# joesharratt1229/DT4Image_Restoration

Hardware: NVIDIA B200
Metric: pnp_admm_image_iters_per_sec_256 (higher is better)
Workload: dtype bf16

## Files before the change

dt4image_restoration_b200/_lib.py:

```python
from __future__ import annotations

import ctypes as C
import os
import threading

_HERE = os.path.dirname(os.path.abspath(__file__))
LIB_PATH = os.path.join(_HERE, "csrc", "libpnp_b200.so")

_lib = None
_inited = False
_init_device = None
_lock = threading.Lock()

c_void_p, c_int, c_ll, c_size_t, c_char_p = C.c_void_p, C.c_int, C.c_longlong, C.c_size_t, C.c_char_p

SIGNATURES = {
    "pnp_init": (c_int, []),
    "pnp_last_error": (c_char_p, []),
    "pnp_num_sms": (c_int, []),
    "pnp_abi_version": (c_int, []),
    "pnp_psnr": (c_int, [c_void_p, c_void_p, c_ll, c_void_p, c_int, c_int, c_void_p]),
    "pnp_psnr_allgather": (c_int, [c_void_p, c_void_p, c_ll, c_void_p, c_void_p, c_int, c_int, c_int, c_int, c_int,
                                   c_void_p, C.c_uint, C.c_uint, c_void_p, c_int, c_int, c_void_p]),
    "pnp_ssim_workspace_bytes": (c_size_t, [c_int, c_int, c_int]),
    "pnp_ssim": (c_int, [c_void_p, c_void_p, c_ll, c_void_p, c_void_p, c_int, c_int, c_int, c_void_p]),
    "pnp_fft2c": (c_int, [c_void_p, c_void_p, c_int, c_int, c_int, c_int, c_void_p]),
    "pnp_simulate_measurements": (c_int, [c_void_p, c_ll, c_void_p, c_ll, c_void_p, c_int, c_void_p, c_void_p, c_void_p,
                                          c_void_p, c_int, c_int, c_int, c_void_p]),
    "pnp_cartesian_masks": (c_int, [c_void_p, c_int, c_void_p, c_int, c_void_p, c_int, c_int, c_int, c_void_p]),
    "pnp_radial_masks": (c_int, [c_void_p, c_int, c_void_p, c_void_p, c_void_p, c_int, c_int, c_int, c_void_p]),
    "pnp_variable_density_masks": (c_int, [c_void_p, c_int, c_void_p, c_int, c_int, c_int, c_void_p, c_int, c_int, c_int,
                                           c_void_p]),
    "pnp_residual_real": (c_int, [c_void_p, c_void_p, c_void_p, c_ll, c_void_p]),
    "pnp_prox_workspace_bytes": (c_size_t, [c_int, c_int, c_int]),
    "pnp_prox_dual": (c_int, [c_void_p, c_void_p, c_void_p, c_void_p, c_ll, c_void_p, c_int, c_void_p, c_void_p,
                              c_void_p, c_void_p, c_int, c_int, c_int, c_void_p]),
    "pnp_prox_prepared_supported": (c_int, [c_int, c_int]),
    "pnp_prox_prepared_bytes": (c_int, [c_int, c_int, c_int, c_void_p, c_void_p]),
    "pnp_prox_prepare": (c_int, [c_void_p, c_void_p, c_ll, c_void_p, c_void_p, c_int, c_int, c_int, c_void_p]),
    "pnp_prox_dual_prepared": (c_int, [c_void_p, c_void_p, c_void_p, c_void_p, c_ll, c_void_p, c_int, c_void_p, c_void_p,
                                       c_void_p, c_int, c_int, c_int, c_void_p]),
    "pnp_prox_prepared_kind_async": (c_int, [c_void_p, c_ll, c_int, c_int, c_int, c_void_p, c_void_p]),
    "pnp_prox_dual_prepared_kind": (c_int, [c_void_p, c_void_p, c_void_p, c_void_p, c_ll, c_void_p, c_int, c_void_p,
                                            c_void_p, c_void_p, c_int, c_int, c_int, c_int, c_void_p]),
    "pnp_step_prepared_kind": (c_int, [c_void_p, c_void_p, c_void_p, c_void_p, c_void_p, c_void_p, c_ll, c_void_p, c_int,
                                       c_void_p, c_void_p, c_void_p, c_void_p, c_int, c_void_p]),
    "pnp_step_prepared_active": (c_int, [c_void_p, c_void_p, c_void_p, c_void_p, c_void_p, c_void_p, c_ll, c_void_p, c_int,
                                         c_void_p, c_void_p, c_void_p, c_void_p, c_int, c_void_p, c_void_p]),
    "pnp_step_prepared": (c_int, [c_void_p, c_void_p, c_void_p, c_void_p, c_void_p, c_void_p, c_ll, c_void_p, c_int,
                                  c_void_p, c_void_p, c_void_p, c_void_p, c_void_p]),
    "pnp_unet_num_params": (c_size_t, []),
    "pnp_unet_packed_bytes": (c_size_t, []),
    "pnp_unet_pack_weights": (c_int, [c_void_p, c_void_p, c_void_p]),
    "pnp_unet_workspace_bytes": (c_size_t, [c_int, c_int, c_int]),
    "pnp_unet_plan_create": (c_int, [C.POINTER(c_void_p), c_void_p, c_void_p, c_size_t, c_int, c_int, c_int]),
    "pnp_unet_plan_destroy": (None, [c_void_p]),
    "pnp_unet_forward": (c_int, [c_void_p, c_void_p, c_void_p, c_void_p, c_void_p, c_void_p]),
    "pnp_unet_profile": (c_int, [c_void_p, c_void_p, c_void_p, c_void_p, c_void_p, C.POINTER(C.c_float),
                                 C.POINTER(c_int), C.POINTER(c_int), C.POINTER(c_int)]),
    "pnp_unet_num_launches": (c_int, [c_void_p]),
    "pnp_unet_micro_batch": (c_int, [c_void_p]),
    "pnp_unet_set_workspace_cap": (c_size_t, [c_size_t]),
    "pnp_unet_set_splitk": (c_int, [c_int]),
    "pnp_unet_plan_tensor": (c_int, [c_void_p, c_char_p, C.POINTER(c_size_t), C.POINTER(c_int), C.POINTER(c_int),
                                     C.POINTER(c_int)]),
    "pnp_conv3x3_packed_bytes": (c_size_t, [c_int, c_int]),
    "pnp_conv3x3_bf16": (c_int, [c_void_p, c_int, c_void_p, c_int, c_void_p, c_void_p, c_void_p, c_void_p, c_int,
                                 c_int, c_int, c_int, c_void_p]),
    "pnp_policy_packed_floats": (c_size_t, [c_int, c_int]),
    "pnp_policy_step": (c_int, [c_void_p, c_void_p, c_void_p, c_void_p, c_void_p, c_void_p, c_void_p, c_void_p, c_void_p,
                                C.c_float, C.c_float, C.c_float, c_int, c_int, c_int, c_int, c_void_p]),
    "pnp_policy_encoder_packed_floats": (c_size_t, []),
    "pnp_policy_observe": (c_int, [c_void_p, c_void_p, c_int, c_int, c_void_p, c_void_p, c_void_p, c_void_p, c_void_p,
                                   c_void_p, c_void_p, c_int, c_int, c_int, c_void_p]),
    "pnp_step": (c_int, [c_void_p, c_void_p, c_void_p, c_void_p, c_void_p, c_void_p, c_ll, c_void_p, c_int, c_void_p,
                         c_void_p, c_void_p, c_void_p, c_void_p, c_void_p]),
}


class PnpError(RuntimeError):
    pass


def load() -> C.CDLL:
    global _lib
    with _lock:
        if _lib is None:
            if not os.path.exists(LIB_PATH):
                raise PnpError(
                    f"{LIB_PATH} is missing: build it with `python -m dt4image_restoration_b200.build` "
                    "(there is no CPU fallback)")
            lib = C.CDLL(LIB_PATH)
            for name, (res, args) in SIGNATURES.items():
                fn = getattr(lib, name)
                fn.restype = res
                fn.argtypes = args
            _lib = lib
    return _lib


def lib() -> C.CDLL:
    global _inited
    l = load()
    if not _inited:
        with _lock:
            if not _inited:
                rc = l.pnp_init()
                if rc != 0:
                    raise PnpError(f"pnp_init failed ({rc}): {l.pnp_last_error().decode()}")
                global _init_device
                try:
                    import torch
                    _init_device = torch.cuda.current_device()
                except Exception:
                    _init_device = None
                _inited = True
    return l


def check_device(device) -> None:
    import torch
    lib()
    idx = torch.device(device).index
    cur = torch.cuda.current_device()
    if idx is None:
        idx = cur
    if _init_device is not None and (idx != _init_device or cur != _init_device):
        raise PnpError(f"libpnp_b200 was initialised on cuda:{_init_device}; got a tensor on cuda:{idx} with current device "
                       f"cuda:{cur}.  Use one process per GPU and call torch.cuda.set_device(local_rank) before the first "
                       f"operation (there is no multi-device dispatch inside one process)")


def check(rc: int, what: str = "") -> None:
    if rc != 0:
        msg = load().pnp_last_error().decode()
        raise PnpError(f"{what or 'libpnp_b200'} failed with code {rc}: {msg}")


def stream_ptr() -> int:
    import torch
    return torch.cuda.current_stream().cuda_stream
```

dt4image_restoration_b200/csrc/api.cu:

```cuda
#include <mutex>
#include <string>
#include "../../include/pnp_b200.h"
#include "common.cuh"
#include "pnp_internal.h"

namespace pnp {
static thread_local std::string t_err;
void set_error(const std::string& msg) { t_err = msg; }
static std::once_flag g_once;
static int g_init_rc = -100;

static int fail_cuda(int rc, const char* where) {
  if (rc > 0 && rc < 1000) set_error(std::string(where) + ": " + cudaGetErrorString(cudaError_t(rc)));
  return rc;
}

__global__ void residual_real_kernel(const float2* __restrict__ z, const float2* __restrict__ u, float* __restrict__ v,
                                     long long n) {
  for (long long i = blockIdx.x * (long long)blockDim.x + threadIdx.x; i < n; i += (long long)gridDim.x * blockDim.x)
    v[i] = z[i].x - u[i].x;
}
}

using namespace pnp;

struct pnp_unet_plan {
  UnetPlan* impl;
  UnetPlan* tail;
  int B, H, W, mb;
};

namespace pnp {
static size_t kUnetWorkspaceCap = size_t(8) << 30;
static int unet_micro_batch(int B, int H, int W) {
  if (unet_workspace_bytes(B, H, W) <= kUnetWorkspaceCap) return B;
  const size_t per8 = unet_workspace_bytes(8, H, W);
  long long m = (long long)(kUnetWorkspaceCap / per8) * 8;
  if (m < 1) m = 1;
  while (m > 1 && unet_workspace_bytes(int(m), H, W) > kUnetWorkspaceCap) m -= (m > 8 ? 8 : 1);
  return int(m < B ? m : B);
}
}

extern "C" {

int pnp_abi_version(void) { return 1; }

int pnp_init(void) {
  std::call_once(g_once, [] {
    int dev = 0;
    cudaError_t e = cudaGetDevice(&dev);
    if (e != cudaSuccess) { g_init_rc = int(e); set_error("no CUDA device"); return; }
    cudaDeviceProp prop;
    cudaGetDeviceProperties(&prop, dev);
    if (prop.major != 10) {
      set_error("libpnp_b200 requires an sm_100a (B200) device; found sm_" + std::to_string(prop.major) +
                std::to_string(prop.minor));
      g_init_rc = -10;
      return;
    }
    init_fft_tables();
    int rc = unet_global_init();
    if (rc == 0) rc = int(cudaGetLastError());
    g_init_rc = rc;
  });
  return g_init_rc;
}

const char* pnp_last_error(void) { return t_err.c_str(); }
int pnp_num_sms(void) { return num_sms(); }

#define REQUIRE_INIT()                                          \
  if (g_init_rc != 0) {                                         \
    set_error("pnp_init() has not succeeded");                  \
    return -3;                                                  \
  }

int pnp_psnr(const float* x, const float* gt, long long gt_batch_stride, float* out, int B, int HW, void* stream) {
  REQUIRE_INIT();
  if (!x || !gt || !out) { set_error("pnp_psnr: null pointer"); return -1; }
  return fail_cuda(psnr_launch(x, gt, gt_batch_stride, out, B, HW, cudaStream_t(stream)), "pnp_psnr");
}

int pnp_psnr_allgather(const float* x, const float* gt, long long gt_batch_stride, float* out_local,
                       const unsigned long long* peer_base, int rank, int world, int slot_floats, int parity,
                       int flag_word, unsigned int* local_count, unsigned int count_target, unsigned int flag_target,
                       int* err_flag, int B, int HW, void* stream) {
  REQUIRE_INIT();
  if (!x || !gt || !peer_base || !local_count || !err_flag) { set_error("pnp_psnr_allgather: null pointer"); return -1; }
  if (world < 1 || world > 8 || rank < 0 || rank >= world || B > slot_floats) {
    set_error("pnp_psnr_allgather: need 1 <= world <= 8, 0 <= rank < world, B <= slot_floats");
    return -1;
  }
  return fail_cuda(psnr_allgather_launch(x, gt, gt_batch_stride, out_local, peer_base, rank, world, slot_floats, parity,
                                         flag_word, local_count, count_target, flag_target, err_flag, B, HW,
                                         cudaStream_t(stream)), "pnp_psnr_allgather");
}

size_t pnp_ssim_workspace_bytes(int B, int H, int W) { return ssim_workspace_bytes(B, H, W); }

int pnp_ssim(const float* x, const float* gt, long long gt_batch_stride, float* out, void* workspace, int B, int H, int W,
             void* stream) {
  REQUIRE_INIT();
  if (!x || !gt || !out || !workspace) { set_error("pnp_ssim: null pointer"); return -1; }
  if (B <= 0) { set_error("pnp_ssim: need B > 0"); return -1; }
  if (H < 11 || W < 11) { set_error("pnp_ssim: H and W must be at least 11 (11x11 window, valid filtering)"); return -2; }
  if (reinterpret_cast<uintptr_t>(workspace) & 15) { set_error("pnp_ssim: workspace must be 16-byte aligned"); return -1; }
  return fail_cuda(ssim_launch(x, gt, gt_batch_stride, out, workspace, B, H, W, cudaStream_t(stream)), "pnp_ssim");
}

int pnp_fft2c(const void* src, void* dst, int B, int H, int W, int inverse, void* stream) {
  REQUIRE_INIT();
  if (!src || !dst || B <= 0) { set_error("pnp_fft2c: bad argument"); return -1; }
  if (!fft_any_shape_supported(H, W)) { set_error("pnp_fft2c: H and W must be in [2, 1024]"); return -2; }
  return fail_cuda(fft2c_general(static_cast<const float2*>(src), static_cast<float2*>(dst), B, H, W, inverse,
                                 cudaStream_t(stream)), "pnp_fft2c");
}

static bool ranges_overlap(const void* a, size_t na, const void* b, size_t nb) {
  const uintptr_t pa = reinterpret_cast<uintptr_t>(a), pb = reinterpret_cast<uintptr_t>(b);
  return a && b && pa < pb + nb && pb < pa + na;
}

int pnp_simulate_measurements(const float* gt, long long gt_batch_stride, const uint8_t* mask, long long mask_batch_stride,
                              const float* sigma_n, int sigma_stride, const unsigned long long* seeds, void* y0_out,
                              void* x0_out, void* aty0_out, int B, int H, int W, void* stream) {
  if (!gt || !mask || !sigma_n || !seeds || !y0_out || !x0_out) {
    set_error("pnp_simulate_measurements: null pointer");
    return -1;
  }
  if (B <= 0 || gt_batch_stride < 0 || mask_batch_stride < 0 || sigma_stride < 0) {
    set_error("pnp_simulate_measurements: need B > 0 and non-negative strides");
    return -1;
  }
  if (!fft_any_shape_supported(H, W)) { set_error("pnp_simulate_measurements: H and W must be in [2, 1024]"); return -2; }
  const size_t hw = size_t(H) * W, nout = size_t(B) * hw * sizeof(float2);
  const size_t ngt = (size_t(B - 1) * gt_batch_stride + hw) * sizeof(float);
  const size_t nmask = size_t(B - 1) * mask_batch_stride + hw;
  const void* outs[3] = {y0_out, x0_out, aty0_out};
  for (int k = 0; k < 3; ++k) {
    bool bad = ranges_overlap(outs[k], nout, gt, ngt) || ranges_overlap(outs[k], nout, mask, nmask);
    for (int q = k + 1; q < 3; ++q) bad |= ranges_overlap(outs[k], nout, outs[q], nout);
    if (bad) { set_error("pnp_simulate_measurements: outputs overlap each other, gt or mask"); return -1; }
  }
  REQUIRE_INIT();
  return fail_cuda(simulate_measurements(gt, gt_batch_stride, mask, mask_batch_stride, sigma_n, sigma_stride, seeds,
                                         static_cast<float2*>(y0_out), static_cast<float2*>(x0_out),
                                         static_cast<float2*>(aty0_out), B, H, W, cudaStream_t(stream)),
                   "pnp_simulate_measurements");
}

int pnp_cartesian_masks(const int* accel, int accel_stride, const unsigned long long* seeds, int acs_cols, uint8_t* mask_out,
                        int B, int H, int W, void* stream) {
  if (!accel || !seeds || !mask_out) { set_error("pnp_cartesian_masks: null pointer"); return -1; }
  if (B <= 0 || accel_stride < 0 || acs_cols < 1) {
    set_error("pnp_cartesian_masks: need B > 0, accel_stride >= 0 and acs_cols >= 1");
    return -1;
  }
  if (!fft_any_shape_supported(H, W)) { set_error("pnp_cartesian_masks: H and W must be in [2, 1024]"); return -2; }
  REQUIRE_INIT();
  return fail_cuda(cartesian_masks(accel, accel_stride, seeds, acs_cols, mask_out, B, H, W, cudaStream_t(stream)),
                   "pnp_cartesian_masks");
}

int pnp_radial_masks(const double* frac, int frac_stride, const unsigned long long* seeds, uint8_t* mask_out,
                     int* lines_out, int B, int H, int W, void* stream) {
  if (!frac || !mask_out) { set_error("pnp_radial_masks: null pointer"); return -1; }
  if (B <= 0 || frac_stride < 0) { set_error("pnp_radial_masks: need B > 0 and frac_stride >= 0"); return -1; }
  if (!fft_any_shape_supported(H, W)) { set_error("pnp_radial_masks: H and W must be in [2, 1024]"); return -2; }
  const size_t nmask = size_t(B) * H * W, nlines = size_t(B) * sizeof(int);
  const size_t nfrac = (size_t(B - 1) * frac_stride + 1) * sizeof(double), nseeds = size_t(B) * sizeof(unsigned long long);
  const bool bad = ranges_overlap(lines_out, nlines, mask_out, nmask) || ranges_overlap(mask_out, nmask, frac, nfrac) ||
                   ranges_overlap(mask_out, nmask, seeds, nseeds) || ranges_overlap(lines_out, nlines, frac, nfrac) ||
                   ranges_overlap(lines_out, nlines, seeds, nseeds);
  if (bad) { set_error("pnp_radial_masks: outputs overlap each other, frac or seeds"); return -1; }
  REQUIRE_INIT();
  return fail_cuda(radial_masks(frac, frac_stride, seeds, mask_out, lines_out, B, H, W, cudaStream_t(stream)),
                   "pnp_radial_masks");
}

int pnp_variable_density_masks(const int* accel, int accel_stride, const unsigned long long* seeds, int acs_h, int acs_w,
                               int power, uint8_t* mask_out, int B, int H, int W, void* stream) {
  if (!accel || !seeds || !mask_out) { set_error("pnp_variable_density_masks: null pointer"); return -1; }
  if (B <= 0 || accel_stride < 0) { set_error("pnp_variable_density_masks: need B > 0 and accel_stride >= 0"); return -1; }
  if (!fft_any_shape_supported(H, W)) { set_error("pnp_variable_density_masks: H and W must be in [2, 1024]"); return -2; }
  if (acs_h < 0 || acs_h > H || acs_w < 0 || acs_w > W || power < 0 || power > 16) {
    set_error("pnp_variable_density_masks: need 0 <= acs_h <= H, 0 <= acs_w <= W and 0 <= power <= 16");
    return -1;
  }
  const size_t nmask = size_t(B) * H * W, nseeds = size_t(B) * sizeof(unsigned long long);
  const size_t naccel = (size_t(B - 1) * accel_stride + 1) * sizeof(int);
  if (ranges_overlap(mask_out, nmask, accel, naccel) || ranges_overlap(mask_out, nmask, seeds, nseeds)) {
    set_error("pnp_variable_density_masks: mask_out overlaps accel or seeds");
    return -1;
  }
  REQUIRE_INIT();
  return fail_cuda(variable_density_masks(accel, accel_stride, seeds, acs_h, acs_w, power, mask_out, B, H, W,
                                          cudaStream_t(stream)), "pnp_variable_density_masks");
}

int pnp_residual_real(const void* z, const void* u, float* v, long long n, void* stream) {
  REQUIRE_INIT();
  long long g = (n + 255) / 256;
  if (g > 148 * 16) g = 148 * 16;
  if (g < 1) g = 1;
  residual_real_kernel<<<int(g), 256, 0, cudaStream_t(stream)>>>(static_cast<const float2*>(z),
                                                                 static_cast<const float2*>(u), v, n);
  return fail_cuda(int(cudaGetLastError()), "pnp_residual_real");
}

size_t pnp_prox_workspace_bytes(int B, int H, int W) { return size_t(B) * H * W * (sizeof(float2) + 1); }

int pnp_prox_prepared_supported(int H, int W) { return fft_shape_supported(H, W); }

int pnp_prox_prepared_bytes(int B, int H, int W, size_t* y0p_bytes, size_t* maskp_bytes) {
  if (!y0p_bytes || !maskp_bytes || B <= 0) { set_error("pnp_prox_prepared_bytes: bad argument"); return -1; }
  if (!pnp_prox_prepared_supported(H, W)) { set_error("pnp_prox_prepared_bytes: H and W must be powers of two in 32..512"); return -2; }
  prox_prepared_bytes(B, H, W, y0p_bytes, maskp_bytes);
  return 0;
}

int pnp_prox_prepare(const void* y0, const uint8_t* mask, long long mask_batch_stride, void* y0T, uint8_t* maskT, int B,
                     int H, int W, void* stream) {
  REQUIRE_INIT();
  if (!y0 || !mask || !y0T || !maskT) { set_error("pnp_prox_prepare: null pointer"); return -1; }
  if (!pnp_prox_prepared_supported(H, W)) { set_error("pnp_prox_prepare: H and W must be powers of two in 32..512"); return -2; }
  return fail_cuda(prox_prepare(static_cast<const float2*>(y0), mask, mask_batch_stride, static_cast<float2*>(y0T), maskT,
                                B, H, W, cudaStream_t(stream)), "pnp_prox_prepare");
}

int pnp_prox_prepared_kind_async(const uint8_t* maskT, long long mask_batch_stride, int B, int H, int W, int* kind_host,
                                 void* stream) {
  REQUIRE_INIT();
  if (!maskT || !kind_host) { set_error("pnp_prox_prepared_kind_async: null pointer"); return -1; }
  if (!pnp_prox_prepared_supported(H, W)) { set_error("pnp_prox_prepared_kind_async: unsupported shape"); return -2; }
  return fail_cuda(int(cudaMemcpyAsync(kind_host, prox_prepared_flag(maskT, mask_batch_stride, B, H, W), sizeof(int),
                                       cudaMemcpyDeviceToHost, cudaStream_t(stream))), "pnp_prox_prepared_kind_async");
}

int pnp_prox_dual_prepared(const float* x, const void* u_in, const void* y0T, const uint8_t* maskT,
                           long long mask_batch_stride, const float* mu, int mu_stride, void* z_out, void* u_out,
                           float* v_next, int B, int H, int W, void* stream) {
  return pnp_prox_dual_prepared_kind(x, u_in, y0T, maskT, mask_batch_stride, mu, mu_stride, z_out, u_out, v_next, B, H, W,
                                     -1, stream);
}

int pnp_prox_dual_prepared_kind(const float* x, const void* u_in, const void* y0T, const uint8_t* maskT,
                                long long mask_batch_stride, const float* mu, int mu_stride, void* z_out, void* u_out,
                                float* v_next, int B, int H, int W, int kind, void* stream) {
  REQUIRE_INIT();
  if (kind < -1 || kind > 1) { set_error("pnp_prox_dual_prepared_kind: kind must be -1, 0 or 1"); return -1; }
  if (!x || !u_in || !y0T || !maskT || !mu || !z_out || !u_out) { set_error("pnp_prox_dual_prepared: null pointer"); return -1; }
  if (!pnp_prox_prepared_supported(H, W)) { set_error("pnp_prox_dual_prepared: H and W must be powers of two in 32..512"); return -2; }
  return fail_cuda(prox_dual_prepared(x, static_cast<const float2*>(u_in), static_cast<const float2*>(y0T), maskT,
                                      mask_batch_stride, mu, mu_stride, static_cast<float2*>(z_out),
                                      static_cast<float2*>(u_out), v_next, B, H, W, kind, cudaStream_t(stream)),
                   "pnp_prox_dual_prepared");
}

int pnp_prox_dual(const float* x, const void* u_in, const void* y0, const uint8_t* mask, long long mask_batch_stride,
                  const float* mu, int mu_stride, void* z_out, void* u_out, float* v_next, void* workspace, int B,
                  int H, int W, void* stream) {
  REQUIRE_INIT();
  if (!x || !u_in || !y0 || !mask || !mu || !z_out || !u_out || !workspace) {
    set_error("pnp_prox_dual: null pointer");
    return -1;
  }
  if (!fft_any_shape_supported(H, W)) {
    set_error("pnp_prox_dual: H and W must be in [2, 1024]");
    return -2;
  }
  return fail_cuda(prox_dual_general(x, static_cast<const float2*>(u_in), static_cast<const float2*>(y0), mask,
                                     mask_batch_stride, mu, mu_stride, static_cast<float2*>(z_out),
                                     static_cast<float2*>(u_out), v_next, static_cast<float2*>(workspace), B, H, W,
                                     cudaStream_t(stream)), "pnp_prox_dual");
}

size_t pnp_unet_num_params(void) { return unet_num_params(); }
size_t pnp_unet_packed_bytes(void) { return unet_packed_bytes(); }
size_t pnp_unet_workspace_bytes(int B, int H, int W) {
  if (B <= 0 || H <= 0 || W <= 0) return 0;
  return unet_workspace_bytes(unet_micro_batch(B, H, W), H, W);
}

int pnp_unet_pack_weights(const float* flat_params, void* packed, void* stream) {
  REQUIRE_INIT();
  return fail_cuda(unet_pack(flat_params, static_cast<uint8_t*>(packed), cudaStream_t(stream)), "pnp_unet_pack_weights");
}

int pnp_unet_plan_create(pnp_unet_plan** plan, const void* packed, void* workspace, size_t workspace_bytes, int B,
                         int H, int W) {
  REQUIRE_INIT();
  if (B <= 0) { set_error("pnp_unet_plan_create: B must be positive"); return -1; }
  const int mb = unet_micro_batch(B, H, W);
  UnetPlan *impl = nullptr, *tail = nullptr;
  int rc = unet_plan_create(&impl, static_cast<const uint8_t*>(packed), static_cast<uint8_t*>(workspace),
                            workspace_bytes, mb, H, W);
  if (rc) return rc;
  if (B % mb) {
    rc = unet_plan_create(&tail, static_cast<const uint8_t*>(packed), static_cast<uint8_t*>(workspace), workspace_bytes,
                          B % mb, H, W);
    if (rc) { unet_plan_destroy(impl); return rc; }
  }
  *plan = new pnp_unet_plan{impl, tail, B, H, W, mb};
  return 0;
}

void pnp_unet_plan_destroy(pnp_unet_plan* plan) {
  if (!plan) return;
  unet_plan_destroy(plan->impl);
  if (plan->tail) unet_plan_destroy(plan->tail);
  delete plan;
}

int pnp_unet_forward(pnp_unet_plan* plan, const float* v, const float* sigma, float* x_out, float* preclamp,
                     void* stream) {
  REQUIRE_INIT();
  if (!plan || !v || !sigma || !x_out) { set_error("pnp_unet_forward: null pointer"); return -1; }
  const size_t hw = size_t(plan->H) * plan->W;
  for (int i0 = 0; i0 < plan->B; i0 += plan->mb) {
    UnetPlan* p = (plan->B - i0 >= plan->mb) ? plan->impl : plan->tail;
    int rc = unet_forward(p, v + i0 * hw, sigma + i0, x_out + i0 * hw, preclamp ? preclamp + i0 * hw : nullptr,
                          cudaStream_t(stream));
    if (rc) return fail_cuda(rc, "pnp_unet_forward");
  }
  return 0;
}

int pnp_unet_profile(pnp_unet_plan* plan, const float* v, const float* sigma, float* x_out, void* stream, float* ms,
                     int* kinds, int* ids, int* n_inout) {
  REQUIRE_INIT();
  if (!plan || !v || !sigma || !x_out || !ms || !kinds || !ids || !n_inout) {
    set_error("pnp_unet_profile: null pointer");
    return -1;
  }
  const size_t hw = size_t(plan->H) * plan->W;
  const int cap = *n_inout;
  int used = 0;
  for (int i0 = 0; i0 < plan->B; i0 += plan->mb) {
    UnetPlan* p = (plan->B - i0 >= plan->mb) ? plan->impl : plan->tail;
    int n = cap - used;
    int rc = unet_profile(p, v + i0 * hw, sigma + i0, x_out + i0 * hw, cudaStream_t(stream), ms + used, kinds + used,
                          ids + used, &n);
    if (rc) return fail_cuda(rc, "pnp_unet_profile");
    used += n;
  }
  *n_inout = used;
  return 0;
}

int pnp_unet_num_launches(const pnp_unet_plan* plan) {
  if (!plan) return -1;
  return (plan->B / plan->mb) * unet_num_launches(plan->impl) + (plan->tail ? unet_num_launches(plan->tail) : 0);
}

int pnp_unet_micro_batch(const pnp_unet_plan* plan) { return plan ? plan->mb : -1; }

size_t pnp_unet_set_workspace_cap(size_t bytes) {
  const size_t old = kUnetWorkspaceCap;
  if (bytes) kUnetWorkspaceCap = bytes;
  return old;
}

int pnp_unet_set_splitk(int mode) { return unet_set_splitk(mode); }

int pnp_unet_plan_tensor(const pnp_unet_plan* plan, const char* name, size_t* byte_offset, int* C, int* H, int* W) {
  if (!plan || !name) return -1;
  if (plan->mb != plan->B) return -1;
  return unet_plan_tensor(plan->impl, name, byte_offset, C, H, W);
}

size_t pnp_policy_packed_floats(int n_time, int n_task) { return policy_packed_floats(n_time, n_task); }

int pnp_policy_step(const float* packed, const float* rtg, const float* emb, float* act, const long long* timesteps,
                    const long long* task, const long long* pos, float* act_out, float* rtg_out, float scale0, float scale1,
                    float scale2, int B, int K, int n_time, int n_task, void* stream) {
  REQUIRE_INIT();
  if (!packed || !rtg || !emb || !act || !timesteps || !task || !pos || !act_out || !rtg_out) {
    set_error("pnp_policy_step: null pointer");
    return -1;
  }
  if (K < 1 || K > 6 || B < 1) { set_error("pnp_policy_step: need 1 <= K <= 6 context entries and B >= 1"); return -1; }
  return fail_cuda(policy_step_launch(packed, rtg, emb, act, timesteps, task, pos, act_out, rtg_out, scale0, scale1, scale2,
                                      B, K, n_time, n_task, cudaStream_t(stream)), "pnp_policy_step");
}

size_t pnp_policy_encoder_packed_floats(void) { return policy_encoder_packed_floats(); }

int pnp_policy_observe(const float* enc_packed, const float* x, int H, int W, const float* next_rtg, float* rtg, float* emb,
                       float* act, long long* timesteps, const long long* pos, const long long* t_dev, int B, int K,
                       int n_time, void* stream) {
  if (!enc_packed || !x || !next_rtg || !rtg || !emb || !act || !timesteps || !pos || !t_dev) {
    set_error("pnp_policy_observe: null pointer");
    return -1;
  }
  if (K < 1 || K > 6 || B < 1 || H != W || H < 128 || H % 128 != 0 || n_time < 1) {
    set_error("pnp_policy_observe: need square images whose edge is a multiple of 128, 1 <= K <= 6 and B >= 1");
    return -1;
  }
  return fail_cuda(policy_observe_launch(enc_packed, x, H, W, next_rtg, rtg, emb, act, timesteps, pos, t_dev, B, K, n_time,
                                         cudaStream_t(stream)), "pnp_policy_observe");
}

size_t pnp_conv3x3_packed_bytes(int Cin, int Cout) { return (conv_packed_bytes(Cin, Cout) + 1023) / 1024 * 1024; }

int pnp_conv3x3_bf16(const void* in0, int C0, const void* in1, int C1, const float* weights, const float* bias,
                     void* out, void* scratch, int B, int H, int W, int Cout, void* stream) {
  REQUIRE_INIT();
  return fail_cuda(conv3x3_single(static_cast<const __nv_bfloat16*>(in0), C0, static_cast<const __nv_bfloat16*>(in1),
                                  C1, weights, bias, static_cast<__nv_bfloat16*>(out), static_cast<uint8_t*>(scratch),
                                  B, H, W, Cout, cudaStream_t(stream)), "pnp_conv3x3_bf16");
}

int pnp_step_prepared(pnp_unet_plan* plan, const float* v, const float* sigma, const void* u_in, const void* y0T,
                      const uint8_t* maskT, long long mask_batch_stride, const float* mu, int mu_stride, float* x_out,
                      void* z_out, void* u_out, float* v_next, void* stream) {
  return pnp_step_prepared_kind(plan, v, sigma, u_in, y0T, maskT, mask_batch_stride, mu, mu_stride, x_out, z_out, u_out,
                                v_next, -1, stream);
}

int pnp_step_prepared_kind(pnp_unet_plan* plan, const float* v, const float* sigma, const void* u_in, const void* y0T,
                           const uint8_t* maskT, long long mask_batch_stride, const float* mu, int mu_stride, float* x_out,
                           void* z_out, void* u_out, float* v_next, int kind, void* stream) {
  int rc = pnp_unet_forward(plan, v, sigma, x_out, nullptr, stream);
  if (rc) return rc;
  return pnp_prox_dual_prepared_kind(x_out, u_in, y0T, maskT, mask_batch_stride, mu, mu_stride, z_out, u_out, v_next,
                                     plan->B, plan->H, plan->W, kind, stream);
}

int pnp_step_prepared_active(pnp_unet_plan* plan, const float* v, const float* sigma, const void* u_in, const void* y0T,
                             const uint8_t* maskT, long long mask_batch_stride, const float* mu, int mu_stride,
                             float* x_out, void* z_out, void* u_out, float* v_next, int kind, const uint8_t* active,
                             void* stream) {
  REQUIRE_INIT();
  if (!plan || !v || !sigma || !u_in || !y0T || !maskT || !mu || !x_out || !z_out || !u_out) {
    set_error("pnp_step_prepared_active: null pointer");
    return -1;
  }
  if (kind < -1 || kind > 1) { set_error("pnp_step_prepared_active: kind must be -1, 0 or 1"); return -1; }
  const size_t hw = size_t(plan->H) * plan->W;
  for (int i0 = 0; i0 < plan->B; i0 += plan->mb) {
    UnetPlan* p = (plan->B - i0 >= plan->mb) ? plan->impl : plan->tail;
    int rc = unet_forward(p, v + i0 * hw, sigma + i0, x_out + i0 * hw, nullptr, cudaStream_t(stream),
                          active ? active + i0 : nullptr);
    if (rc) return fail_cuda(rc, "pnp_step_prepared_active");
  }
  return fail_cuda(prox_dual_prepared(x_out, static_cast<const float2*>(u_in), static_cast<const float2*>(y0T), maskT,
                                      mask_batch_stride, mu, mu_stride, static_cast<float2*>(z_out),
                                      static_cast<float2*>(u_out), v_next, plan->B, plan->H, plan->W, kind,
                                      cudaStream_t(stream), active), "pnp_step_prepared_active");
}

int pnp_step(pnp_unet_plan* plan, const float* v, const float* sigma, const void* u_in, const void* y0,
             const uint8_t* mask, long long mask_batch_stride, const float* mu, int mu_stride, float* x_out,
             void* z_out, void* u_out, float* v_next, void* prox_workspace, void* stream) {
  int rc = pnp_unet_forward(plan, v, sigma, x_out, nullptr, stream);
  if (rc) return rc;
  return pnp_prox_dual(x_out, u_in, y0, mask, mask_batch_stride, mu, mu_stride, z_out, u_out, v_next, prox_workspace,
                       plan->B, plan->H, plan->W, stream);
}

}
```

dt4image_restoration_b200/csrc/pnp_internal.h:

```cpp
#pragma once
#include <cuda_runtime.h>
#include <cuda_bf16.h>
#include <stddef.h>
#include <stdint.h>
#include <string>

namespace pnp {

void set_error(const std::string& msg);

int psnr_launch(const float* x, const float* gt, long long gt_bstride, float* out, int B, int HW, cudaStream_t st);
int psnr_allgather_launch(const float* x, const float* gt, long long gt_bstride, float* out_local,
                          const unsigned long long* peer_base, int rank, int world, int slot, int parity, int flag_word,
                          unsigned int* local_count, unsigned int count_target, unsigned int flag_target, int* err,
                          int B, int HW, cudaStream_t st);

size_t ssim_workspace_bytes(int B, int H, int W);
int ssim_launch(const float* x, const float* gt, long long gt_bstride, float* out, void* workspace, int B, int H, int W,
                cudaStream_t st);

void init_fft_tables();
int fft_shape_supported(int H, int W);
int fft_any_shape_supported(int H, int W);
int prox_dual_general(const float* x, const float2* u_in, const float2* y0, const uint8_t* mask,
                      long long mask_bstride, const float* mu, int mu_stride, float2* z_out, float2* u_out,
                      float* v_out, float2* work, int B, int H, int W, cudaStream_t st);
void prox_prepared_bytes(int B, int H, int W, size_t* y0p_bytes, size_t* maskp_bytes);
int prox_prepare(const float2* y0, const uint8_t* mask, long long mask_bstride, float2* y0T, uint8_t* maskT, int B, int H,
                 int W, cudaStream_t st);
int prox_dual_prepared(const float* x, const float2* u_in, const float2* y0T, const uint8_t* maskT,
                       long long mask_bstride, const float* mu, int mu_stride, float2* z_out, float2* u_out,
                       float* v_out, int B, int H, int W, int kind, cudaStream_t st, const uint8_t* active = nullptr);
const int* prox_prepared_flag(const uint8_t* maskp, long long mask_bstride, int B, int H, int W);
int fft2c_general(const float2* src, float2* dst, int B, int H, int W, int inverse, cudaStream_t st);
int simulate_measurements(const float* gt, long long gt_bstride, const uint8_t* mask, long long mask_bstride,
                          const float* sigma, int sigma_stride, const unsigned long long* seeds, float2* y0, float2* x0,
                          float2* aty0, int B, int H, int W, cudaStream_t st);
int cartesian_masks(const int* accel, int accel_stride, const unsigned long long* seeds, int acs_cols, uint8_t* mask,
                    int B, int H, int W, cudaStream_t st);
int radial_masks(const double* frac, int frac_stride, const unsigned long long* seeds, uint8_t* mask, int* lines_out,
                 int B, int H, int W, cudaStream_t st);
int variable_density_masks(const int* accel, int accel_stride, const unsigned long long* seeds, int acs_h, int acs_w,
                           int power, uint8_t* mask, int B, int H, int W, cudaStream_t st);

size_t policy_packed_floats(int n_time, int n_task);
int policy_step_launch(const float* w, const float* rtg, const float* emb, float* act, const long long* ts,
                       const long long* task, const long long* pos, float* act_out, float* rtg_out, float s0, float s1,
                       float s2, int B, int K, int n_time, int n_task, cudaStream_t st);
size_t policy_encoder_packed_floats();
int policy_observe_launch(const float* w, const float* x, int H, int W, const float* nxt_rtg, float* w_rtg, float* w_emb,
                          float* w_act, long long* w_ts, const long long* pos, const long long* t_dev, int B, int K,
                          int n_time, cudaStream_t st);

struct UnetPlan;
int unet_global_init();
int num_sms();
size_t unet_num_params();
size_t unet_packed_bytes();
size_t unet_workspace_bytes(int B, int H, int W);
int unet_pack(const float* flat_fp32, uint8_t* packed, cudaStream_t st);
int unet_plan_create(UnetPlan** out, const uint8_t* packed, uint8_t* workspace, size_t workspace_bytes, int B, int H,
                     int W);
void unet_plan_destroy(UnetPlan* p);
int unet_plan_tensor(const UnetPlan* p, const char* name, size_t* off, int* C, int* H, int* W);
int unet_forward(UnetPlan* p, const float* v, const float* sigma, float* x_out, float* preclamp, cudaStream_t st,
                 const uint8_t* active = nullptr);
int unet_profile(UnetPlan* p, const float* v, const float* sigma, float* x_out, cudaStream_t st, float* ms, int* kinds,
                 int* ids, int* n_inout);
int unet_num_launches(const UnetPlan* p);
int unet_set_splitk(int mode);
size_t conv_packed_bytes(int Cin, int Cout);
int conv3x3_single(const __nv_bfloat16* in0, int C0, const __nv_bfloat16* in1, int C1, const float* w_fp32,
                   const float* bias, __nv_bfloat16* out, uint8_t* wpk_scratch, int B, int H, int W, int Cout,
                   cudaStream_t st);

}
```

dt4image_restoration_b200/csrc/unet.cu:

```cuda
#include <algorithm>
#include <mutex>
#include <vector>
#include <string>
#include <cstring>
#include "common.cuh"
#include "unet_conv.cuh"
#include "unet_conv_kws.cuh"
#include "unet_conv_pair.cuh"
#include "unet_conv_splitk.cuh"
#include "pnp_internal.h"

namespace pnp {

struct FirstConvW {
  float w[9][32];
  float b[32];
  float ws[9][32];
};


__global__ void __launch_bounds__(256) conv_first_kernel(const float* __restrict__ v, const float* __restrict__ sigma,
                                                         const __grid_constant__ FirstConvW cw,
                                                         __nv_bfloat16* __restrict__ out, int B, int H, int W,
                                                         float slope, int rev, int ppt) {
  grid_dep_launch();
  grid_dep_wait();
  const int x = blockIdx.x * blockDim.x + threadIdx.x;
  const int pairs = (H + 1) / 2;
  const int pair0 = ppt * (rev ? int(gridDim.y) - 1 - int(blockIdx.y) : int(blockIdx.y));
  const int pair1 = pair0 + ppt < pairs ? pair0 + ppt : pairs;
  const int b = rev ? B - 1 - int(blockIdx.z) : int(blockIdx.z);
  if (x >= W) return;
  const float sg = __ldg(sigma + b);
  const float* vb = v + size_t(b) * H * W + x;
  const bool xl = x > 0, xr = x + 1 < W;
  const int cx = xl ? (xr ? 1 : 2) : 0;
  auto load_row = [&](int yy, float (&r)[3]) {
    const bool ok = (yy >= 0) && (yy < H);
    const float* row = vb + ptrdiff_t(yy) * W;
    r[0] = (ok && xl) ? __ldg(row - 1) : 0.f;
    r[1] = ok ? __ldg(row) : 0.f;
    r[2] = (ok && xr) ? __ldg(row + 1) : 0.f;
  };
  float in[4][3], nx[2][3];
#pragma unroll
  for (int r = 0; r < 4; ++r) load_row(2 * pair0 - 1 + r, in[r]);
#pragma unroll 1
  for (int pair = pair0; pair < pair1; ++pair) {
    const int y0 = 2 * pair;
    load_row(y0 + 3, nx[0]);
    load_row(y0 + 4, nx[1]);
    const int cs0 = (y0 == 0 ? 0 : (y0 == H - 1 ? 6 : 3)) + cx;
    const int cs1 = (y0 + 1 == H - 1 ? 6 : 3) + cx;
    float acc0[32], acc1[32];
    if (cs0 == 4 && cs1 == 4) {
#pragma unroll
      for (int co = 0; co < 32; ++co) acc0[co] = acc1[co] = fmaf(sg, cw.ws[4][co], cw.b[co]);
    } else {
#pragma unroll
      for (int co = 0; co < 32; ++co) {
        acc0[co] = fmaf(sg, cw.ws[cs0][co], cw.b[co]);
        acc1[co] = fmaf(sg, cw.ws[cs1][co], cw.b[co]);
      }
    }
#pragma unroll
    for (int t = 0; t < 9; ++t) {
#pragma unroll
      for (int co = 0; co < 32; ++co) {
        const float wv = cw.w[t][co];
        acc0[co] = fmaf(wv, in[t / 3][t % 3], acc0[co]);
        acc1[co] = fmaf(wv, in[t / 3 + 1][t % 3], acc1[co]);
      }
    }
#pragma unroll
    for (int p = 0; p < 2; ++p) {
      if (p == 1 && y0 + 1 >= H) break;
      const float* acc = p ? acc1 : acc0;
      uint32_t o[16];
#pragma unroll
      for (int co = 0; co < 32; co += 2) {
        const float a0 = fmaxf(acc[co], acc[co] * slope);
        const float a1 = fmaxf(acc[co + 1], acc[co + 1] * slope);
        o[co / 2] = pack_bf16x2(a0, a1);
      }
      uint4* dst = reinterpret_cast<uint4*>(out + ((size_t(b) * H + y0 + p) * W + x) * 32);
      dst[0] = make_uint4(o[0], o[1], o[2], o[3]);
      dst[1] = make_uint4(o[4], o[5], o[6], o[7]);
      dst[2] = make_uint4(o[8], o[9], o[10], o[11]);
      dst[3] = make_uint4(o[12], o[13], o[14], o[15]);
    }
#pragma unroll
    for (int c = 0; c < 3; ++c) {
      in[0][c] = in[2][c]; in[1][c] = in[3][c]; in[2][c] = nx[0][c]; in[3][c] = nx[1][c];
    }
  }
}


constexpr int kUpsRows = 4;
__global__ void __launch_bounds__(256) upsample2x_kernel(const uint4* __restrict__ in, uint4* __restrict__ out, int B,
                                                         int h, int w, int Ho, int Wo, int C8, int py, int px,
                                                         float sy, float sx) {
  grid_dep_launch();
  grid_dep_wait();
  const int e = blockIdx.x * blockDim.x + threadIdx.x;
  if (e >= Wo * C8) return;
  const int c = e % C8, xo = e / C8;
  const int b = blockIdx.z;
  const int ux = xo - px;
  const bool xin = ux >= 0 && ux < 2 * w;
  const float fx = sx * float(ux);
  const int x0 = xin ? int(fx) : 0;
  const int x1 = x0 + (x0 < w - 1 ? 1 : 0);
  const float lx = fx - float(x0), hx = 1.f - lx;
  const size_t base = size_t(b) * h * w;
  uint4 q[kUpsRows][4];
  float ly[kUpsRows];
  bool ok[kUpsRows];
#pragma unroll
  for (int r = 0; r < kUpsRows; ++r) {
    const int yo = blockIdx.y * kUpsRows + r;
    const int uy = yo - py;
    ok[r] = xin && yo < Ho && uy >= 0 && uy < 2 * h;
    const float fy = sy * float(uy);
    const int y0 = ok[r] ? int(fy) : 0;
    const int y1 = y0 + (y0 < h - 1 ? 1 : 0);
    ly[r] = fy - float(y0);
    q[r][0] = __ldg(in + (base + size_t(y0) * w + x0) * C8 + c);
    q[r][1] = __ldg(in + (base + size_t(y0) * w + x1) * C8 + c);
    q[r][2] = __ldg(in + (base + size_t(y1) * w + x0) * C8 + c);
    q[r][3] = __ldg(in + (base + size_t(y1) * w + x1) * C8 + c);
  }
#pragma unroll
  for (int r = 0; r < kUpsRows; ++r) {
    const int yo = blockIdx.y * kUpsRows + r;
    if (yo >= Ho) break;
    uint4 res = make_uint4(0, 0, 0, 0);
    if (ok[r]) {
      const float hy = 1.f - ly[r];
      const __nv_bfloat162* a = reinterpret_cast<const __nv_bfloat162*>(&q[r][0]);
      const __nv_bfloat162* bq = reinterpret_cast<const __nv_bfloat162*>(&q[r][1]);
      const __nv_bfloat162* cq = reinterpret_cast<const __nv_bfloat162*>(&q[r][2]);
      const __nv_bfloat162* d = reinterpret_cast<const __nv_bfloat162*>(&q[r][3]);
      uint32_t* o = reinterpret_cast<uint32_t*>(&res);
#pragma unroll
      for (int k = 0; k < 4; ++k) {
        const float2 f00 = __bfloat1622float2(a[k]), f01 = __bfloat1622float2(bq[k]);
        const float2 f10 = __bfloat1622float2(cq[k]), f11 = __bfloat1622float2(d[k]);
        const float vx = hy * (hx * f00.x + lx * f01.x) + ly[r] * (hx * f10.x + lx * f11.x);
        const float vy = hy * (hx * f00.y + lx * f01.y) + ly[r] * (hx * f10.y + lx * f11.y);
        o[k] = pack_bf16x2(vx, vy);
      }
    }
    out[(size_t(b) * Ho + yo) * Wo * C8 + e] = res;
  }
}

__device__ __forceinline__ float small_int_to_float(int k) { return __int_as_float(0x4B000000 + (k + 1)) - 8388609.0f; }


__global__ void __launch_bounds__(256) upsample2x_fast_kernel(const uint4* __restrict__ in, uint4* __restrict__ out,
                                                              int h, int w, int C8, float sy, float sx, int nimg,
                                                              int rev, int c8_shift, int walk) {
  grid_dep_launch();
  grid_dep_wait();
  const int e = blockIdx.x * blockDim.x + threadIdx.x;
  if (e >= (w + 1) * C8) return;
  const int c = e & (C8 - 1), n = (e >> c8_shift) - 1;
  const int by = rev ? int(gridDim.y) - 1 - int(blockIdx.y) : int(blockIdx.y);
  const int m0 = by * walk - 1;
  const int m1 = (m0 + walk < h) ? m0 + walk : h;
  const int b = rev ? nimg - 1 - int(blockIdx.z) : int(blockIdx.z);
  const int xa = n < 0 ? 0 : n, xb = n + 1 < w ? n + 1 : w - 1;
  const uint4* src = in + size_t(b) * h * w * C8 + c;
  const int Ho = 2 * h, Wo = 2 * w;
  float lx[2];
#pragma unroll
  for (int j = 0; j < 2; ++j) lx[j] = sx * small_int_to_float(2 * n + 1 + j) - small_int_to_float(n);
  auto xlerp = [&](const uint4& qa, const uint4& qb, float2 (&t)[2][4]) {
    const uint32_t* a = reinterpret_cast<const uint32_t*>(&qa);
    const uint32_t* bb = reinterpret_cast<const uint32_t*>(&qb);
#pragma unroll
    for (int k = 0; k < 4; ++k) {
      const float2 fa = make_float2(__uint_as_float(a[k] << 16), __uint_as_float(a[k] & 0xffff0000u));
      const float2 fb = make_float2(__uint_as_float(bb[k] << 16), __uint_as_float(bb[k] & 0xffff0000u));
#pragma unroll
      for (int j = 0; j < 2; ++j) {
        const float2 l2 = make_float2(lx[j], lx[j]), h2 = make_float2(1.f - lx[j], 1.f - lx[j]);
        t[j][k] = __ffma2_rn(fb, l2, __fmul2_rn(fa, h2));
      }
    }
  };
  auto row_ptr = [&](int y) { return src + size_t(y < 0 ? 0 : (y < h ? y : h - 1)) * w * C8; };
  float2 top[2][4], bot[2][4];
  {
    const uint4* r = row_ptr(m0);
    xlerp(__ldg(r + size_t(xa) * C8), __ldg(r + size_t(xb) * C8), top);
  }
  const uint4* rn = row_ptr(m0 + 1);
  uint4 qa = __ldg(rn + size_t(xa) * C8), qb = __ldg(rn + size_t(xb) * C8);
#pragma unroll 1
  for (int m = m0; m < m1; ++m) {
    xlerp(qa, qb, bot);
    if (m + 1 < m1) {
      rn = row_ptr(m + 2);
      qa = __ldg(rn + size_t(xa) * C8); qb = __ldg(rn + size_t(xb) * C8);
    }
#pragma unroll
    for (int i = 0; i < 2; ++i) {
      const int yo = 2 * m + 1 + i;
      if (yo < 0 || yo >= Ho) continue;
      const float ly = sy * small_int_to_float(yo) - small_int_to_float(m);
      const float2 ll = make_float2(ly, ly), hh = make_float2(1.f - ly, 1.f - ly);
#pragma unroll
      for (int j = 0; j < 2; ++j) {
        const int xo = 2 * n + 1 + j;
        if (xo < 0 || xo >= Wo) continue;
        uint4 res;
#pragma unroll
        for (int k = 0; k < 4; ++k) {
          const float2 v = __ffma2_rn(bot[j][k], ll, __fmul2_rn(top[j][k], hh));
          reinterpret_cast<uint32_t*>(&res)[k] = pack_bf16x2(v.x, v.y);
        }
        out[((size_t(b) * Ho + yo) * Wo + xo) * C8 + c] = res;
      }
    }
#pragma unroll
    for (int j = 0; j < 2; ++j)
#pragma unroll
      for (int k = 0; k < 4; ++k) top[j][k] = bot[j][k];
  }
}

__global__ void pack_weights_kernel(const float* __restrict__ w, uint8_t* __restrict__ out, int Cin, int Cout, int KC,
                                    int BN) {
  const int n_tiles = Cout / BN;
  const int ROWB = KC * 2;
  const int swz_mask = (ROWB == 128) ? 7 : 3;
  const size_t total = size_t(Cout) * Cin * 9;
  for (size_t i = size_t(blockIdx.x) * blockDim.x + threadIdx.x; i < total; i += size_t(gridDim.x) * blockDim.x) {
    const int tap = int(i % 9);
    const int ci = int((i / 9) % Cin);
    const int co = int(i / (size_t(9) * Cin));
    const int chunk = ci / KC, kk = ci % KC;
    const int nt = co / BN, n = co % BN;
    const uint32_t off = uint32_t(n * ROWB + (kk / 8) * 16);
    const uint32_t phys = off ^ (((off >> 7) & swz_mask) << 4);
    const size_t blob = (size_t(chunk) * 9 + tap) * n_tiles + nt;
    __nv_bfloat16* dst = reinterpret_cast<__nv_bfloat16*>(out + blob * size_t(BN) * ROWB + phys) + (kk % 8);
    *dst = __float2bfloat16_rn(w[i]);
  }
}

__global__ void pack_weights_kws_kernel(const float* __restrict__ w, uint8_t* __restrict__ out, int Cin) {
  const size_t total = size_t(32) * Cin * 9;
  for (size_t i = size_t(blockIdx.x) * blockDim.x + threadIdx.x; i < total; i += size_t(gridDim.x) * blockDim.x) {
    const int tap = int(i % 9), kh = tap / 3, kw = tap % 3;
    const int ci = int((i / 9) % Cin);
    const int co = int(i / (size_t(9) * Cin));
    const int chunk = ci / 32, kk = ci % 32;
    const int n = kw * 32 + co;
    const uint32_t off = uint32_t(n * 64 + (kk / 8) * 16);
    const uint32_t phys = off ^ (((off >> 7) & 3) << 4);
    const size_t blob = size_t(chunk) * 3 + kh;
    __nv_bfloat16* dst = reinterpret_cast<__nv_bfloat16*>(out + blob * size_t(KwsCfg::B_BYTES) + phys) + (kk % 8);
    *dst = __float2bfloat16_rn(w[i]);
  }
}

typedef CUresult (*EncodeTiledFn)(CUtensorMap*, CUtensorMapDataType, cuuint32_t, void*, const cuuint64_t*,
                                  const cuuint64_t*, const cuuint32_t*, const cuuint32_t*, CUtensorMapInterleave,
                                  CUtensorMapSwizzle, CUtensorMapL2promotion, CUtensorMapFloatOOBfill);
static EncodeTiledFn g_encode = nullptr;
static int g_num_sms = 148;
static const int kSkGain = 3;
static int g_splitk_mode = -1;
int unet_set_splitk(int mode) {
  const int old = g_splitk_mode;
  if (mode >= -1 && mode <= 1) g_splitk_mode = mode;
  return old;
}

static const int kConvSmemMax = 227 * 1024;
static const int kConvSmemBudget = 222 * 1024;

template <int KC, int BN, int EPI>
static int set_conv_attr() {
  return int(cudaFuncSetAttribute(conv3x3_umma_kernel<KC, BN, EPI>, cudaFuncAttributeMaxDynamicSharedMemorySize,
                                  kConvSmemMax));
}

int unet_global_init() {
  void* fn = nullptr;
  cudaDriverEntryPointQueryResult qres;
  cudaError_t e = cudaGetDriverEntryPoint("cuTensorMapEncodeTiled", &fn, cudaEnableDefault, &qres);
  if (e != cudaSuccess || fn == nullptr) {
    set_error("cuTensorMapEncodeTiled driver entry point not available");
    return e != cudaSuccess ? int(e) : 999;
  }
  g_encode = reinterpret_cast<EncodeTiledFn>(fn);
  int dev = 0;
  cudaGetDevice(&dev);
  cudaDeviceGetAttribute(&g_num_sms, cudaDevAttrMultiProcessorCount, dev);
  int rc = 0;
  rc |= set_conv_attr<32, 32, EPI_BF16>();
  rc |= set_conv_attr<32, 32, EPI_FINAL>();
  rc |= set_conv_attr<32, 64, EPI_BF16>();
  rc |= set_conv_attr<64, 64, EPI_BF16>();
  rc |= set_conv_attr<64, 128, EPI_BF16>();
  rc |= int(cudaFuncSetAttribute(conv3x3_pair_kernel<32, 64>, cudaFuncAttributeMaxDynamicSharedMemorySize, kConvSmemMax));
  rc |= int(cudaFuncSetAttribute(conv3x3_pair_kernel<64, 64>, cudaFuncAttributeMaxDynamicSharedMemorySize, kConvSmemMax));
  rc |= int(cudaFuncSetAttribute(conv3x3_pair_kernel<64, 128>, cudaFuncAttributeMaxDynamicSharedMemorySize, kConvSmemMax));
  rc |= int(cudaFuncSetAttribute(conv3x3_kws_kernel, cudaFuncAttributeMaxDynamicSharedMemorySize, kConvSmemMax));
  rc |= int(cudaFuncSetAttribute(conv3x3_splitk_kernel, cudaFuncAttributeMaxDynamicSharedMemorySize, kSkSmem));
  if (rc) set_error("cudaFuncSetAttribute(MaxDynamicSharedMemorySize) failed");
  return rc;
}

int num_sms() { return g_num_sms; }

static int make_act_map(CUtensorMap* m, const void* base, int B, int H, int W, int C, int KC, int box_w = kHalo,
                        int box_h = kHalo) {
  if (!g_encode) { set_error("pnp_init() has not been called"); return -3; }
  cuuint64_t dims[4] = {cuuint64_t(C), cuuint64_t(W), cuuint64_t(H), cuuint64_t(B)};
  cuuint64_t strides[3] = {cuuint64_t(C) * 2, cuuint64_t(W) * C * 2, cuuint64_t(H) * W * C * 2};
  cuuint32_t box[4] = {cuuint32_t(KC), cuuint32_t(box_w), cuuint32_t(box_h), 1};
  cuuint32_t estr[4] = {1, 1, 1, 1};
  CUresult r = g_encode(m, CU_TENSOR_MAP_DATA_TYPE_BFLOAT16, 4, const_cast<void*>(base), dims, strides, box, estr,
                        CU_TENSOR_MAP_INTERLEAVE_NONE, KC == 64 ? CU_TENSOR_MAP_SWIZZLE_128B : CU_TENSOR_MAP_SWIZZLE_64B,
                        CU_TENSOR_MAP_L2_PROMOTION_L2_128B, CU_TENSOR_MAP_FLOAT_OOB_FILL_NONE);
  if (r != CUDA_SUCCESS) {
    set_error("cuTensorMapEncodeTiled failed (code " + std::to_string(int(r)) + ")");
    return 1000 + int(r);
  }
  return 0;
}

struct ConvLaunch {
  ConvParams p;
  CUtensorMap tm0, tm1;
  CUtensorMap tmw;
  int KC, BN, EPI;
  int kws;
  int pair;
  int splitk;
  int grid;
  int smem;
};

static const int kConvBarBytes = (4 * 16 + 2 * 4 + 2) * 8 + 16 + kEpiSmemFloats * 4;
static const int kConvRingBytes = kConvSmemBudget - 1024 - kConvBarBytes - 1024;
static int halo_stage_bytes(int KC) { return (kHalo * kHalo * KC * 2 + 1023) / 1024 * 1024; }

static bool weights_fit(int KC, int n_tiles, long long wbytes) {
  return n_tiles == 1 && wbytes + 3 * halo_stage_bytes(KC) <= kConvRingBytes;
}

static void size_rings(ConvLaunch& L) {
  if (L.kws) {
    const int bar = KwsCfg::BAR_BYTES;
    const int avail = kConvSmemBudget - 1024 - bar - 1024;
    const int wtotal = (L.p.nchunks0 + L.p.nchunks1) * 3 * KwsCfg::B_BYTES;
    int sa = (avail - wtotal) / KwsCfg::A_STAGE;
    L.p.wres = 1; L.p.sb = 1;
    L.p.sa = sa > 8 ? 8 : sa;
    L.smem = 1024 + L.p.sa * KwsCfg::A_STAGE + ((wtotal + 1023) & ~1023) + bar;
    return;
  }
  const int ROWB = L.KC * 2;
  const int a_stage = halo_stage_bytes(L.KC);
  const int b_bytes = L.BN * ROWB / (L.pair ? 2 : 1);
  const int b_stage = (b_bytes + 1023) / 1024 * 1024;
  const int bar = kConvBarBytes;
  const int avail = kConvRingBytes;
  const int nchunks = L.p.nchunks0 + L.p.nchunks1;
  const int wtotal = nchunks * 9 * b_bytes;
  ConvParams& p = L.p;
  if (weights_fit(L.KC, p.n_tiles, wtotal)) {
    p.wres = 1;
    p.sb = 1;
    int sa = (avail - wtotal) / a_stage;
    p.sa = sa > 8 ? 8 : sa;
    L.smem = 1024 + p.sa * a_stage + ((wtotal + 1023) & ~1023) + bar;
  } else {
    p.wres = 0;
    p.sa = 2;
    int sb = (avail - p.sa * a_stage) / b_stage;
    if (sb > 12) sb = 12;
    if (sb < 2) { p.sa = 2; sb = (avail - p.sa * a_stage) / b_stage; }
    p.sb = sb;
    L.smem = 1024 + p.sa * a_stage + p.sb * b_stage + bar;
  }
}

static int pick_bn(int Cout) { return Cout >= 128 ? 128 : Cout; }

static bool use_kws(int C0, int C1, int Cout) {
  return Cout == 32 && C0 > 0 && C0 % 32 == 0 && C1 % 32 == 0 && (C0 + C1) >= 64 && (C0 + C1) <= 96;
}

size_t conv_packed_bytes(int Cin, int Cout) { return size_t(Cin) * Cout * 9 * 2; }

static int build_conv(ConvLaunch& L, const __nv_bfloat16* in0, int C0, const __nv_bfloat16* in1, int C1,
                      const uint8_t* wpk, const float* bias, __nv_bfloat16* out, int B, int H, int W, int Cout,
                      int epi) {
  const bool kws = use_kws(C0, C1, Cout);
  const int KC = (!kws && C0 % 64 == 0 && C1 % 64 == 0) ? 64 : 32;
  if (C0 % KC || C1 % KC || C0 <= 0) { set_error("conv: channel counts must be multiples of 32"); return -4; }
  const int BN = pick_bn(Cout);
  if (Cout % BN) { set_error("conv: Cout must be 32, 64 or a multiple of 128"); return -4; }
  if (epi == EPI_FINAL && !(KC == 32 && BN == 32)) { set_error("conv: FINAL epilogue needs Cin=Cout=32"); return -4; }
  L = ConvLaunch{};
  L.KC = KC; L.BN = BN; L.EPI = epi; L.kws = kws ? 1 : 0;
  {
    static const int pair_env = [] { const char* e = getenv("PNP_CONV_PAIR"); return e ? atoi(e) : -1; }();
    const bool eligible = !kws && epi == EPI_BF16 && (BN == 64 || BN == 128);
    const bool want = pair_env < 0 ? !weights_fit(KC, Cout / BN, (long long)(C0 + C1) * 9 * BN * 2) : pair_env == 1;
    L.pair = (eligible && want) ? 1 : 0;
  }
  ConvParams& p = L.p;
  {
    const long long pix_tiles = (long long)B * ((W + kTile - 1) / kTile) * ((H + kTile - 1) / kTile);
    const bool eligible = !kws && epi == EPI_BF16 && KC == 64 && Cout % kSkBN == 0;
    const long long units = pix_tiles * (Cout / kSkBN);
    if (eligible && g_splitk_mode != 0 && (units <= g_num_sms || g_splitk_mode == 1) && units < (1ll << 24)) {
      const int nch = (C0 + C1) / kSkKC;
      int S = 8;
      while (S > 1 && (nch % S != 0 || units * S > g_num_sms)) S >>= 1;
      const long long reg_ctas = std::min<long long>(pix_tiles * (Cout / BN), g_num_sms);
      if (g_splitk_mode == 1 || units * S >= kSkGain * reg_ctas) {
        L.splitk = 1; L.pair = 0;
        p.sk_split = S; p.sk_cpc = nch / S; p.sk_stages = p.sk_cpc < kSkStages ? p.sk_cpc : kSkStages;
      }
    }
  }
  p.B = B; p.H = H; p.W = W;
  p.tiles_x = kws ? (W + kKwsTileW - 1) / kKwsTileW : (W + kTile - 1) / kTile;
  p.tiles_y = kws ? (H + kKwsTileH - 1) / kKwsTileH : (H + kTile - 1) / kTile;
  p.n_tiles = Cout / BN;
  p.nchunks0 = C0 / KC; p.nchunks1 = C1 / KC;
  p.Cout = Cout; p.wpk = wpk; p.bias = bias; p.out = out; p.slope = 0.2f;
  p.mg_n = conv_magic(uint32_t(p.n_tiles)); p.mg_x = conv_magic(uint32_t(p.tiles_x)); p.mg_y = conv_magic(uint32_t(p.tiles_y));
  {
    const long long tiles_all = (long long)B * p.tiles_x * p.tiles_y * p.n_tiles;
    const int dmax = std::max(p.n_tiles, std::max(p.tiles_x, p.tiles_y));
    if (tiles_all * dmax >= (1ll << 32) || Cout > 512) { set_error("conv: problem too large for the tile index arithmetic"); return -4; }
  }
  size_rings(L);
  const int bw = kws ? kKwsHaloW : kHalo, bh = kws ? kKwsHaloH : kHalo;
  int rc = make_act_map(&L.tm0, in0, B, H, W, C0, KC, bw, bh);
  if (rc) return rc;
  rc = C1 > 0 ? make_act_map(&L.tm1, in1, B, H, W, C1, KC, bw, bh) : make_act_map(&L.tm1, in0, B, H, W, C0, KC, bw, bh);
  if (rc) return rc;
  if (L.pair) {
    const cuuint64_t rows = cuuint64_t(p.nchunks0 + p.nchunks1) * 9 * Cout;
    cuuint64_t dims[2] = {cuuint64_t(KC), rows};
    cuuint64_t strides[1] = {cuuint64_t(KC) * 2};
    cuuint32_t box[2] = {cuuint32_t(KC), cuuint32_t(BN / 2)};
    cuuint32_t estr[2] = {1, 1};
    CUresult r = g_encode(&L.tmw, CU_TENSOR_MAP_DATA_TYPE_BFLOAT16, 2, const_cast<uint8_t*>(wpk), dims, strides, box, estr,
                          CU_TENSOR_MAP_INTERLEAVE_NONE, CU_TENSOR_MAP_SWIZZLE_NONE, CU_TENSOR_MAP_L2_PROMOTION_L2_128B,
                          CU_TENSOR_MAP_FLOAT_OOB_FILL_NONE);
    if (r != CUDA_SUCCESS) { set_error("cuTensorMapEncodeTiled (weights) failed (code " + std::to_string(int(r)) + ")"); return 1000 + int(r); }
  }
  long long tiles = (long long)B * p.tiles_x * p.tiles_y * p.n_tiles;
  if (L.pair) {
    const long long pix = (long long)B * p.tiles_x * p.tiles_y;
    tiles = (pix + 1) / 2 * p.n_tiles;
    p.total_tiles = int(tiles);
    const long long pairs = g_num_sms / 2;
    L.grid = 2 * int(tiles < pairs ? tiles : pairs);
  } else {
  p.total_tiles = int(tiles);
  L.grid = int(tiles < g_num_sms ? tiles : g_num_sms);
  }
  if (L.splitk) {
    L.grid = int((long long)B * p.tiles_x * p.tiles_y * (Cout / kSkBN) * p.sk_split);
    L.smem = sk_smem_bytes(p.sk_stages);
  }
  return 0;
}

template <typename... KArgs, typename... Args>
static cudaError_t launch_k(void (*kernel)(KArgs...), dim3 grid, dim3 block, size_t smem, cudaStream_t st, Args&&... args) {
  cudaLaunchConfig_t cfg{};
  cfg.gridDim = grid; cfg.blockDim = block; cfg.dynamicSmemBytes = smem; cfg.stream = st;
  cudaLaunchAttribute attr[1];
  attr[0].id = cudaLaunchAttributeProgrammaticStreamSerialization;
  attr[0].val.programmaticStreamSerializationAllowed = 1;
  cfg.attrs = attr;
  cfg.numAttrs = 1;
  return cudaLaunchKernelEx(&cfg, kernel, KArgs(args)...);
}

template <int KC, int BN, int EPI>
static void launch_conv_t(const ConvLaunch& L, cudaStream_t st) {
  launch_k(conv3x3_umma_kernel<KC, BN, EPI>, dim3(L.grid), dim3(kConvThreads), size_t(L.smem), st, L.p, L.tm0, L.tm1);
}

static int launch_conv(const ConvLaunch& L, cudaStream_t st) {
  if (L.splitk) {
    cudaLaunchConfig_t cfg{};
    cfg.gridDim = dim3(L.grid); cfg.blockDim = dim3(kConvThreads); cfg.dynamicSmemBytes = size_t(L.smem); cfg.stream = st;
    cudaLaunchAttribute attr[2];
    attr[0].id = cudaLaunchAttributeClusterDimension;
    attr[0].val.clusterDim.x = unsigned(L.p.sk_split); attr[0].val.clusterDim.y = 1; attr[0].val.clusterDim.z = 1;
    attr[1].id = cudaLaunchAttributeProgrammaticStreamSerialization;
    attr[1].val.programmaticStreamSerializationAllowed = 1;
    cfg.attrs = attr; cfg.numAttrs = 2;
    return int(cudaLaunchKernelEx(&cfg, conv3x3_splitk_kernel, L.p, L.tm0, L.tm1));
  }
  if (L.pair) {
    if (L.KC == 32 && L.BN == 64)
      launch_k(conv3x3_pair_kernel<32, 64>, dim3(L.grid), dim3(kConvThreads), size_t(L.smem), st, L.p, L.tm0, L.tm1, L.tmw);
    else if (L.KC == 64 && L.BN == 64)
      launch_k(conv3x3_pair_kernel<64, 64>, dim3(L.grid), dim3(kConvThreads), size_t(L.smem), st, L.p, L.tm0, L.tm1, L.tmw);
    else if (L.KC == 64 && L.BN == 128)
      launch_k(conv3x3_pair_kernel<64, 128>, dim3(L.grid), dim3(kConvThreads), size_t(L.smem), st, L.p, L.tm0, L.tm1, L.tmw);
    else { set_error("conv: unsupported (KC,BN) combination for the pair kernel"); return -4; }
    return int(cudaGetLastError());
  }
  if (L.kws) {
    launch_k(conv3x3_kws_kernel, dim3(L.grid), dim3(kConvThreads), size_t(L.smem), st, L.p, L.tm0, L.tm1);
    return int(cudaGetLastError());
  }
  if (L.EPI == EPI_FINAL) launch_conv_t<32, 32, EPI_FINAL>(L, st);
  else if (L.KC == 32 && L.BN == 32) launch_conv_t<32, 32, EPI_BF16>(L, st);
  else if (L.KC == 32 && L.BN == 64) launch_conv_t<32, 64, EPI_BF16>(L, st);
  else if (L.KC == 64 && L.BN == 64) launch_conv_t<64, 64, EPI_BF16>(L, st);
  else if (L.KC == 64 && L.BN == 128) launch_conv_t<64, 128, EPI_BF16>(L, st);
  else { set_error("conv: unsupported (KC,BN) combination"); return -4; }
  return int(cudaGetLastError());
}

static int ew_grid(size_t total) {
  size_t g = (total + 255) / 256;
  const size_t cap = size_t(g_num_sms) * 16;
  return int(g < cap ? (g ? g : 1) : cap);
}

int pack_conv_weights(const float* w_fp32, uint8_t* out, int Cin, int Cout, int KC, cudaStream_t st, bool kws) {
  if (kws) {
    pack_weights_kws_kernel<<<ew_grid(size_t(Cin) * Cout * 9), 256, 0, st>>>(w_fp32, out, Cin);
    return int(cudaGetLastError());
  }
  const int BN = pick_bn(Cout);
  pack_weights_kernel<<<ew_grid(size_t(Cin) * Cout * 9), 256, 0, st>>>(w_fp32, out, Cin, Cout, KC, BN);
  return int(cudaGetLastError());
}

int conv3x3_single(const __nv_bfloat16* in0, int C0, const __nv_bfloat16* in1, int C1, const float* w_fp32,
                   const float* bias, __nv_bfloat16* out, uint8_t* wpk_scratch, int B, int H, int W, int Cout,
                   cudaStream_t st) {
  ConvLaunch L;
  int rc = build_conv(L, in0, C0, in1, C1, wpk_scratch, bias, out, B, H, W, Cout, EPI_BF16);
  if (rc) return rc;
  rc = pack_conv_weights(w_fp32, wpk_scratch, C0 + C1, Cout, L.KC, st, L.kws != 0);
  if (rc) return rc;
  return launch_conv(L, st);
}

static const int kCh[5] = {32, 64, 128, 256, 512};

struct TensorSlot { size_t off; int C, H, W; };

enum { K_FIRST = 0, K_UMMA = 1, K_UPS = 3 };

struct Op {
  int kind;
  int id;
  int level;
  int conv;
  int rev;
};

struct UnetPlan {
  int B, H, W;
  int Hl[5], Wl[5];
  uint8_t* ws;
  size_t ws_bytes;
  const uint8_t* wts;
  TensorSlot tA[5], tB[5], skip[5], pooled[5], ups[4];
  std::vector<ConvLaunch> convs;
  std::vector<Op> ops;
  FirstConvW first;
};

struct LayerDesc { int cin, cout; size_t w_off, b_off; size_t pk_off; };
static const int kBlockCin[9] = {2, 32, 64, 128, 256, 768, 384, 192, 96};
static const int kBlockCout[9] = {32, 64, 128, 256, 512, 256, 128, 64, 32};

static void layer_table(LayerDesc (&L)[27], size_t& outc_w, size_t& outc_b, size_t& n_params, size_t& pk_bytes) {
  size_t off = 0, pk = 0;
  for (int blk = 0; blk < 9; ++blk)
    for (int i = 0; i < 3; ++i) {
      LayerDesc& d = L[blk * 3 + i];
      d.cin = (i == 0) ? kBlockCin[blk] : kBlockCout[blk];
      d.cout = kBlockCout[blk];
      d.w_off = off; off += size_t(d.cout) * d.cin * 9;
      d.b_off = off; off += d.cout;
      d.pk_off = pk;
      if (blk * 3 + i > 0) pk += (conv_packed_bytes(d.cin, d.cout) + 1023) / 1024 * 1024;
    }
  outc_w = off; off += 32;
  outc_b = off; off += 1;
  n_params = off;
  pk_bytes = pk;
}

size_t unet_num_params() {
  LayerDesc L[27]; size_t a, b, n, pk;
  layer_table(L, a, b, n, pk);
  return n;
}
size_t unet_packed_bytes() {
  LayerDesc L[27]; size_t a, b, n, pk;
  layer_table(L, a, b, n, pk);
  return pk + (n * sizeof(float) + 1023) / 1024 * 1024;
}

int unet_pack(const float* flat_fp32, uint8_t* packed, cudaStream_t st) {
  LayerDesc L[27]; size_t ow, ob, n, pk;
  layer_table(L, ow, ob, n, pk);
  for (int i = 1; i < 27; ++i) {
    const int cin = L[i].cin, cout = L[i].cout;
    int c0 = cin, c1 = 0;
    if (i >= 15 && i % 3 == 0) { c0 = kBlockCout[i / 3]; c1 = cin - c0; }
    const bool kws = use_kws(c0, c1, cout);
    const int KC = (!kws && c0 % 64 == 0 && c1 % 64 == 0) ? 64 : 32;
    int rc = pack_conv_weights(flat_fp32 + L[i].w_off, packed + L[i].pk_off, cin, cout, KC, st, kws);
    if (rc) return rc;
  }
  return int(cudaMemcpyAsync(packed + pk, flat_fp32, n * sizeof(float), cudaMemcpyDeviceToDevice, st));
}

static size_t plan_layout(UnetPlan* P) {
  size_t off = 0;
  auto take = [&](TensorSlot& s, int C, int H, int W) {
    s.off = off; s.C = C; s.H = H; s.W = W;
    off += (size_t(P->B) * H * W * C * 2 + 1023) / 1024 * 1024;
  };
  for (int l = 0; l < 5; ++l) {
    take(P->tA[l], kCh[l], P->Hl[l], P->Wl[l]);
    take(P->tB[l], kCh[l], P->Hl[l], P->Wl[l]);
    take(P->skip[l], kCh[l], P->Hl[l], P->Wl[l]);
    if (l > 0) take(P->pooled[l], kCh[l - 1], P->Hl[l], P->Wl[l]);
    if (l < 4) take(P->ups[l], kCh[l + 1], P->Hl[l], P->Wl[l]);
  }
  return off;
}

size_t unet_workspace_bytes(int B, int H, int W) {
  UnetPlan P{};
  P.B = B; P.H = H; P.W = W;
  for (int l = 0; l < 5; ++l) { P.Hl[l] = H >> l; P.Wl[l] = W >> l; }
  return plan_layout(&P);
}

int unet_plan_create(UnetPlan** out, const uint8_t* packed, uint8_t* workspace, size_t workspace_bytes, int B, int H,
                     int W) {
  if (B <= 0 || H < 16 || W < 16) { set_error("unet plan: need B>0 and H,W >= 16"); return -1; }
  UnetPlan* P = new UnetPlan();
  P->B = B; P->H = H; P->W = W;
  for (int l = 0; l < 5; ++l) { P->Hl[l] = H >> l; P->Wl[l] = W >> l; }
  const size_t need = plan_layout(P);
  if (workspace_bytes < need) { delete P; set_error("unet plan: workspace too small"); return -5; }
  if ((reinterpret_cast<uintptr_t>(workspace) & 1023) || (reinterpret_cast<uintptr_t>(packed) & 1023)) {
    delete P; set_error("unet plan: workspace / packed weights must be 1024-byte aligned"); return -6;
  }
  P->ws = workspace; P->ws_bytes = workspace_bytes; P->wts = packed;
  LayerDesc L[27]; size_t ow, ob, n, pk;
  layer_table(L, ow, ob, n, pk);
  const float* flat = reinterpret_cast<const float*>(packed + pk);
  auto T = [&](const TensorSlot& s) { return reinterpret_cast<__nv_bfloat16*>(P->ws + s.off); };
  int rc = 0;
  auto conv = [&](int li, const TensorSlot& in0, const TensorSlot* in1, const TensorSlot& o, int lvl,
                  const TensorSlot* pooled = nullptr) {
    if (rc) return;
    ConvLaunch cl;
    const int epi = (li == 26) ? EPI_FINAL : EPI_BF16;
    rc = build_conv(cl, T(in0), in0.C, in1 ? T(*in1) : nullptr, in1 ? in1->C : 0, packed + L[li].pk_off,
                    flat + L[li].b_off, T(o), B, P->Hl[lvl], P->Wl[lvl], L[li].cout, epi);
    if (rc) return;
    if (epi == EPI_FINAL) { cl.p.wout = flat + ow; cl.p.bout = flat + ob; }
    if (pooled) cl.p.pool_out = T(*pooled);
    P->convs.push_back(cl);
    P->ops.push_back(Op{K_UMMA, li, lvl, int(P->convs.size()) - 1});
  };
  {
    float hw[32 * 18 + 32];
    cudaError_t e = cudaMemcpy(hw, flat + L[0].w_off, sizeof(hw), cudaMemcpyDeviceToHost);
    if (e != cudaSuccess) { delete P; set_error("unet plan: cannot read first-layer weights"); return int(e); }
    for (int co = 0; co < 32; ++co) {
      for (int k = 0; k < 9; ++k) P->first.w[k][co] = hw[co * 18 + k];
      P->first.b[co] = hw[32 * 18 + co];
      for (int cy = 0; cy < 3; ++cy)
        for (int cx = 0; cx < 3; ++cx) {
          float t = 0.f;
          for (int k = 0; k < 9; ++k) {
            const int dy = k / 3 - 1, dx = k % 3 - 1;
            const bool in_y = !((cy == 0 && dy < 0) || (cy == 2 && dy > 0));
            const bool in_x = !((cx == 0 && dx < 0) || (cx == 2 && dx > 0));
            if (in_y && in_x) t += hw[co * 18 + 9 + k];
          }
          P->first.ws[cy * 3 + cx][co] = t;
        }
    }
  }
  P->ops.push_back(Op{K_FIRST, 0, 0, -1});
  conv(1, P->tA[0], nullptr, P->tB[0], 0);
  conv(2, P->tB[0], nullptr, P->skip[0], 0, &P->pooled[1]);
  for (int l = 1; l <= 4; ++l) {
    conv(l * 3 + 0, P->pooled[l], nullptr, P->tA[l], l);
    conv(l * 3 + 1, P->tA[l], nullptr, P->tB[l], l);
    conv(l * 3 + 2, P->tB[l], nullptr, P->skip[l], l, l < 4 ? &P->pooled[l + 1] : nullptr);
  }
  for (int l = 3; l >= 0; --l) {
    const int blk = 5 + (3 - l);
    P->ops.push_back(Op{K_UPS, 200 + l, l, -1});
    conv(blk * 3 + 0, P->skip[l], &P->ups[l], P->tA[l], l);
    conv(blk * 3 + 1, P->tA[l], nullptr, P->tB[l], l);
    conv(blk * 3 + 2, P->tB[l], nullptr, P->tA[l], l);
  }
  if (rc) { delete P; return rc; }
  {
    int k = 0;
    for (Op& op : P->ops) {
      op.rev = k & 1;
      if (op.kind == K_UMMA) P->convs[op.conv].p.rev = op.rev;
      ++k;
    }
  }
  *out = P;
  return 0;
}

void unet_plan_destroy(UnetPlan* P) { delete P; }

int unet_plan_tensor(const UnetPlan* P, const char* name, size_t* off, int* C, int* H, int* W) {
  const TensorSlot* s = nullptr;
  const std::string n(name);
  if (n == "inc.conv-0") s = &P->tA[0];
  else if (n == "inc.conv-1") s = &P->tB[0];
  else if (n == "inc.conv-2") s = &P->skip[0];
  else {
    for (int l = 1; l <= 4 && !s; ++l) {
      const std::string d = "down" + std::to_string(l);
      if (n == d + ".pooled") s = &P->pooled[l];
      else if (n == d + ".conv-0") s = &P->tA[l];
      else if (n == d + ".conv-1") s = &P->tB[l];
      else if (n == d + ".conv-2") s = &P->skip[l];
    }
    for (int k = 1; k <= 4 && !s; ++k) {
      const int l = 4 - k;
      const std::string u = "up" + std::to_string(k);
      if (n == u + ".upsampled") s = &P->ups[l];
    }
  }
  if (!s) return -1;
  *off = s->off; *C = s->C; *H = s->H; *W = s->W;
  return 0;
}

struct ProfileCtx {
  std::vector<cudaEvent_t> ev;
  cudaStream_t st;
  void begin() {
    cudaEvent_t a, b;
    cudaEventCreate(&a); cudaEventCreate(&b);
    ev.push_back(a); ev.push_back(b);
    cudaEventRecord(a, st);
  }
  void end() { cudaEventRecord(ev.back(), st); }
};

static int unet_forward_impl(UnetPlan* P, const float* v, const float* sigma, float* x_out, float* preclamp,
                             cudaStream_t st, ProfileCtx* prof, const uint8_t* active = nullptr) {
  LayerDesc L[27]; size_t ow, ob, n, pk;
  layer_table(L, ow, ob, n, pk);
  auto T = [&](const TensorSlot& s) { return reinterpret_cast<__nv_bfloat16*>(P->ws + s.off); };
  int rc = 0;
  for (const Op& op : P->ops) {
    if (prof) prof->begin();
    switch (op.kind) {
      case K_FIRST: {
        const int bd = P->W >= 256 ? 256 : ((P->W + 31) / 32) * 32;
        const int gx = (P->W + bd - 1) / bd, pairs = (P->H + 1) / 2;
        int ppt = 4;
        while (ppt > 1 && size_t(gx) * ((pairs + ppt - 1) / ppt) * P->B < 4 * 148) ppt >>= 1;
        launch_k(conv_first_kernel, dim3(gx, (pairs + ppt - 1) / ppt, P->B), dim3(bd), 0, st, v, sigma, P->first,
                 T(P->tA[0]), P->B, P->H, P->W, 0.2f, op.rev, ppt);
        break;
      }
      case K_UMMA: {
        ConvLaunch& cl = P->convs[op.conv];
        if (cl.EPI == EPI_FINAL) { cl.p.noisy = v; cl.p.x_out = x_out; cl.p.preclamp = preclamp; cl.p.active = active; }
        rc = launch_conv(cl, st);
        break;
      }
      case K_UPS: {
        const int l = op.level;
        const TensorSlot& lo = (l == 3) ? P->skip[4] : P->tA[l + 1];
        const int h = P->Hl[l + 1], w = P->Wl[l + 1], Ho = P->Hl[l], Wo = P->Wl[l];
        const int C8 = kCh[l + 1] / 8;
        const int dy = Ho - 2 * h, dx = Wo - 2 * w;
        const float sy = (2 * h > 1) ? float(h - 1) / float(2 * h - 1) : 0.f;
        const float sx = (2 * w > 1) ? float(w - 1) / float(2 * w - 1) : 0.f;
        if (dy == 0 && dx == 0 && h > 1 && w > 1)
        {
          const int gx = ((w + 1) * C8 + 255) / 256;
          int walk = 8;
          while (walk > 1 && size_t(gx) * ((h + walk) / walk) * P->B < 4 * size_t(g_num_sms)) walk >>= 1;
          launch_k(upsample2x_fast_kernel, dim3(gx, (h + walk) / walk, P->B), dim3(256), 0, st,
                   reinterpret_cast<const uint4*>(T(lo)), reinterpret_cast<uint4*>(T(P->ups[l])), h, w,
                   C8, sy, sx, P->B, op.rev, (C8 == 64 ? 6 : (C8 == 32 ? 5 : (C8 == 16 ? 4 : 3))), walk);
        }
        else
          launch_k(upsample2x_kernel, dim3((Wo * C8 + 255) / 256, (Ho + kUpsRows - 1) / kUpsRows, P->B), dim3(256), 0,
                   st, reinterpret_cast<const uint4*>(T(lo)), reinterpret_cast<uint4*>(T(P->ups[l])),
                   P->B, h, w, Ho, Wo, C8, dy / 2, dx / 2, sy, sx);
        break;
      }
    }
    if (prof) prof->end();
    if (rc) return rc;
  }
  return int(cudaGetLastError());
}

int unet_forward(UnetPlan* P, const float* v, const float* sigma, float* x_out, float* preclamp, cudaStream_t st,
                 const uint8_t* active) {
  return unet_forward_impl(P, v, sigma, x_out, preclamp, st, nullptr, active);
}

int unet_num_launches(const UnetPlan* P) { return int(P->ops.size()); }

int unet_profile(UnetPlan* P, const float* v, const float* sigma, float* x_out, cudaStream_t st, float* ms,
                 int* kinds, int* ids, int* n_inout) {
  ProfileCtx prof;
  prof.st = st;
  int rc = unet_forward_impl(P, v, sigma, x_out, nullptr, st, &prof);
  cudaError_t e = cudaStreamSynchronize(st);
  const int n = int(prof.ev.size() / 2);
  const int cap = *n_inout;
  for (int i = 0; i < n && i < cap; ++i) {
    float t = 0.f;
    cudaEventElapsedTime(&t, prof.ev[2 * i], prof.ev[2 * i + 1]);
    ms[i] = t; kinds[i] = P->ops[i].kind; ids[i] = P->ops[i].id;
  }
  for (cudaEvent_t evt : prof.ev) cudaEventDestroy(evt);
  *n_inout = n < cap ? n : cap;
  if (rc) return rc;
  return int(e);
}

}
```

dt4image_restoration_b200/csrc/unet_conv_pair.cuh:

```cuda
#pragma once
#include <cooperative_groups.h>
#include "unet_conv.cuh"

namespace pnp {
namespace cgp = cooperative_groups;

__device__ __forceinline__ void tmem_alloc2(uint32_t* smem_dst, uint32_t ncols) {
  asm volatile("tcgen05.alloc.cta_group::2.sync.aligned.shared::cta.b32 [%0], %1;" ::"r"(smem_u32(smem_dst)), "r"(ncols)
               : "memory");
}
__device__ __forceinline__ void tmem_relinquish2() {
  asm volatile("tcgen05.relinquish_alloc_permit.cta_group::2.sync.aligned;" ::: "memory");
}
__device__ __forceinline__ void tmem_dealloc2(uint32_t taddr, uint32_t ncols) {
  asm volatile("tcgen05.dealloc.cta_group::2.sync.aligned.b32 %0, %1;" ::"r"(taddr), "r"(ncols) : "memory");
}
__device__ __forceinline__ void tc_commit2(uint64_t* bar) {
  asm volatile("tcgen05.commit.cta_group::2.mbarrier::arrive::one.shared::cluster.multicast::cluster.b64 [%0], %1;" ::"r"(
                   smem_u32(bar)),
               "h"(uint16_t(3))
               : "memory");
}
__device__ __forceinline__ void umma2_bf16_ss(uint32_t tmem_d, uint32_t a_lo, uint32_t a_hi, uint32_t b_lo, uint32_t b_hi,
                                              uint32_t idesc, uint32_t accumulate) {
  asm volatile(
      "{\n\t.reg .pred p;\n\t.reg .b64 da, db;\n\t"
      "mov.b64 da, {%1, %2};\n\t"
      "mov.b64 db, {%3, %4};\n\t"
      "setp.ne.b32 p, %6, 0;\n\t"
      "tcgen05.mma.cta_group::2.kind::f16 [%0], da, db, %5, p;\n\t}\n" ::"r"(tmem_d),
      "r"(a_lo), "r"(a_hi), "r"(b_lo), "r"(b_hi), "r"(idesc), "r"(accumulate)
      : "memory");
}
__device__ __forceinline__ uint32_t cluster_addr(const void* p, uint32_t rank) {
  uint32_t ra;
  asm volatile("mapa.shared::cluster.u32 %0, %1, %2;" : "=r"(ra) : "r"(smem_u32(p)), "r"(rank));
  return ra;
}
__device__ __forceinline__ void tma_load_4d_pair(void* smem_dst, const CUtensorMap* m, uint32_t mbar_cluster, int c0, int c1,
                                                 int c2, int c3) {
  asm volatile(
      "cp.async.bulk.tensor.4d.cta_group::2.shared::cluster.global.mbarrier::complete_tx::bytes [%0], [%1, {%3, %4, %5, %6}], [%2];"
      ::"r"(smem_u32(smem_dst)), "l"(reinterpret_cast<uint64_t>(m)), "r"(mbar_cluster), "r"(c0), "r"(c1), "r"(c2), "r"(c3)
      : "memory");
}
__device__ __forceinline__ void tma_load_2d_pair(void* smem_dst, const CUtensorMap* m, uint32_t mbar_cluster, int c0, int c1) {
  asm volatile(
      "cp.async.bulk.tensor.2d.cta_group::2.shared::cluster.global.mbarrier::complete_tx::bytes [%0], [%1, {%3, %4}], [%2];"
      ::"r"(smem_u32(smem_dst)), "l"(reinterpret_cast<uint64_t>(m)), "r"(mbar_cluster), "r"(c0), "r"(c1)
      : "memory");
}
__device__ __forceinline__ void mbar_arrive_remote(uint64_t* bar, uint32_t rank) {
  asm volatile(
      "{\n\t.reg .b32 ra;\n\t"
      "mapa.shared::cluster.u32 ra, %0, %1;\n\t"
      "mbarrier.arrive.relaxed.cluster.shared::cluster.b64 _, [ra];\n\t}\n" ::"r"(smem_u32(bar)),
      "r"(rank)
      : "memory");
}

template <int KC, int BN>
struct PairCfg {
  static constexpr int ROWB = KC * 2;
  static constexpr int A_BYTES = kHalo * kHalo * ROWB;
  static constexpr int A_STAGE = (A_BYTES + 1023) / 1024 * 1024;
  static constexpr int B_FULL = BN * ROWB;
  static constexpr int B_BYTES = B_FULL / 2;
  static constexpr int B_STAGE = (B_BYTES + 1023) / 1024 * 1024;
  static constexpr int NACC = 2;
  static constexpr int TMEM_COLS = 2 * BN * NACC;
  static constexpr int MAX_RING = 16;
  static constexpr int BAR_BYTES = (4 * MAX_RING + 2 * NACC + 2) * 8 + 16 + kEpiSmemFloats * 4;
  static_assert(TMEM_COLS >= 32 && TMEM_COLS <= 512 && (TMEM_COLS & (TMEM_COLS - 1)) == 0, "TMEM cols");
  static_assert((BN / 2) % 8 == 0, "half blobs must be whole 8-row groups");
};

template <int KC, int BN>
__global__ void __cluster_dims__(2, 1, 1) __launch_bounds__(kConvThreads, 1)
conv3x3_pair_kernel(const ConvParams p, const __grid_constant__ CUtensorMap tmA0,
                    const __grid_constant__ CUtensorMap tmA1, const __grid_constant__ CUtensorMap tmW) {
  using Cfg = PairCfg<KC, BN>;
  constexpr int ROWB = Cfg::ROWB;
  constexpr int NACC = Cfg::NACC;
  const int SA = p.sa, SB = p.sb;
  const int nchunks = p.nchunks0 + p.nchunks1;
  const int b_region = p.wres ? nchunks * 9 * Cfg::B_BYTES : SB * Cfg::B_STAGE;

  extern __shared__ uint8_t smem_raw[];
  uint8_t* smem = reinterpret_cast<uint8_t*>((reinterpret_cast<uintptr_t>(smem_raw) + 1023) & ~uintptr_t(1023));
  uint8_t* a_smem = smem;
  uint8_t* b_smem = smem + SA * Cfg::A_STAGE;
  uint64_t* bars = reinterpret_cast<uint64_t*>(b_smem + ((b_region + 1023) & ~1023));
  uint64_t* a_full = bars;
  uint64_t* a_empty = a_full + Cfg::MAX_RING;
  uint64_t* b_full = a_empty + Cfg::MAX_RING;
  uint64_t* b_empty = b_full + Cfg::MAX_RING;
  uint64_t* acc_full = b_empty + Cfg::MAX_RING;
  uint64_t* acc_empty = acc_full + NACC;
  uint64_t* w_full = acc_empty + NACC;
  uint32_t* tmem_slot = reinterpret_cast<uint32_t*>(w_full + 2);
  float* epi_s = reinterpret_cast<float*>(tmem_slot + 4);

  cgp::cluster_group cluster = cgp::this_cluster();
  const uint32_t rank = cluster.block_rank();
  const bool leader = rank == 0;
  const int warp = threadIdx.x >> 5;
  const int lane = threadIdx.x & 31;
  const int pixel_tiles = p.B * p.tiles_y * p.tiles_x;
  const int total_pairs = p.total_tiles;
  const int pair_id = int(blockIdx.x) >> 1, n_pairs = int(gridDim.x) >> 1;

  grid_dep_launch();
  if (warp == 0 && lane == 0) {
    tma_prefetch_desc(&tmA0);
    tma_prefetch_desc(&tmA1);
    tma_prefetch_desc(&tmW);
  }
  if (warp == 1 && lane == 0) {
    for (int i = 0; i < SA; ++i) { mbar_init(&a_full[i], 1); mbar_init(&a_empty[i], kNumMmaWarps); }
    for (int i = 0; i < SB; ++i) { mbar_init(&b_full[i], 1); mbar_init(&b_empty[i], kNumMmaWarps); }
    for (int i = 0; i < NACC; ++i) { mbar_init(&acc_full[i], kNumMmaWarps); mbar_init(&acc_empty[i], 2 * kNumEpiWarps); }
    mbar_init(w_full, 1);
    fence_mbar_init();
  }
  if (warp == 2) {
    tmem_alloc2(tmem_slot, Cfg::TMEM_COLS);
    tmem_relinquish2();
  }
  if (warp >= kEpiWarp0) {
    const int t = threadIdx.x - kEpiWarp0 * 32;
    for (int i = t; i < p.Cout; i += kNumEpiWarps * 32) epi_s[i] = __ldg(p.bias + i);
  }
  tc_fence_before();
  cluster.sync();
  tc_fence_after();
  const uint32_t tmem_base = *tmem_slot;

  auto my_tile = [&](int u, int& nt, int& tx, int& ty, int& img, bool& dup) {
    const int uu = p.rev ? total_pairs - 1 - u : u;
    nt = uu % p.n_tiles;
    int pt = 2 * (uu / p.n_tiles) + int(rank);
    dup = pt >= pixel_tiles;
    if (dup) pt = pixel_tiles - 1;
    tx = pt % p.tiles_x; pt /= p.tiles_x;
    ty = pt % p.tiles_y;
    img = pt / p.tiles_y;
  };

  if (warp == 0) {
    if (lane == 0) {
      int sa = 0, pa = 0, sb = 0, pb = 0;
      const int row_half = int(rank) * (BN / 2);
      if (p.wres && pair_id < total_pairs) {
        const uint32_t wbar = cluster_addr(w_full, 0);
        if (leader) mbar_arrive_expect_tx(w_full, 2u * uint32_t(nchunks) * 9 * Cfg::B_BYTES);
        for (int i = 0; i < nchunks * 9; ++i)
          tma_load_2d_pair(b_smem + size_t(i) * Cfg::B_BYTES, &tmW, wbar, 0, i * BN + row_half);
      }
      grid_dep_wait();
      for (int u = pair_id; u < total_pairs; u += n_pairs) {
        int nt, tx, ty, img; bool dup;
        my_tile(u, nt, tx, ty, img, dup);
        for (int c = 0; c < nchunks; ++c) {
          mbar_wait(&a_empty[sa], pa ^ 1);
          if (leader) mbar_arrive_expect_tx(&a_full[sa], 2u * Cfg::A_BYTES);
          const bool seg0 = c < p.nchunks0;
          tma_load_4d_pair(a_smem + sa * Cfg::A_STAGE, seg0 ? &tmA0 : &tmA1, cluster_addr(&a_full[sa], 0),
                           (seg0 ? c : c - p.nchunks0) * KC, tx * kTile - 1, ty * kTile - 1, img);
          if (++sa == SA) { sa = 0; pa ^= 1; }
          if (p.wres) continue;
          const int row0 = (c * 9 * p.n_tiles + nt) * BN + row_half;
          for (int tap = 0; tap < 9; ++tap) {
            mbar_wait(&b_empty[sb], pb ^ 1);
            if (leader) mbar_arrive_expect_tx(&b_full[sb], 2u * Cfg::B_BYTES);
            tma_load_2d_pair(b_smem + sb * Cfg::B_STAGE, &tmW, cluster_addr(&b_full[sb], 0), 0,
                             row0 + tap * p.n_tiles * BN);
            if (++sb == SB) { sb = 0; pb ^= 1; }
          }
        }
      }
    }
  } else if (leader && (warp == 1 || warp == 3)) {
    const int mb = warp == 3 ? 1 : 0;
    constexpr uint32_t idesc = umma_idesc_bf16(256, BN);
    constexpr uint32_t kLayout = (ROWB == 128) ? 2u : 4u;
    constexpr uint32_t a_hi = (uint32_t(kHalo * ROWB) >> 4) | (1u << 14) | (kLayout << 29);
    constexpr uint32_t b_hi = (uint32_t(8 * ROWB) >> 4) | (1u << 14) | (kLayout << 29);
    int sa = 0, pa = 0, sb = 0, pb = 0;
    int it = 0;
    if (p.wres && pair_id < total_pairs) mbar_wait(w_full, 0);
    for (int u = pair_id; u < total_pairs; u += n_pairs, ++it) {
      const int as = it % NACC;
      const uint32_t aph = (it / NACC) & 1;
      mbar_wait(&acc_empty[as], aph ^ 1);
      const uint32_t d0 = tmem_base + as * (2 * BN) + mb * BN;
      for (int c = 0; c < nchunks; ++c) {
        mbar_wait(&a_full[sa], pa);
        tc_fence_after();
        const uint32_t a_lo0 = ((smem_u32(a_smem + sa * Cfg::A_STAGE) + uint32_t(mb * 8 * ROWB)) >> 4) | (1u << 16);
        if (p.wres) {
          const uint32_t b_lo0 = (smem_u32(b_smem + c * 9 * Cfg::B_BYTES) >> 4) | (1u << 16);
          if (elect_one()) {
#pragma unroll
            for (int tap = 0; tap < 9; ++tap) {
              const uint32_t a_tap = a_lo0 + uint32_t(((tap / 3) * kHalo + (tap % 3)) * ROWB) / 16;
              const uint32_t b_tap = b_lo0 + uint32_t(tap * Cfg::B_BYTES) / 16;
#pragma unroll
              for (int k = 0; k < KC / 16; ++k)
                umma2_bf16_ss(d0, a_tap + k * 2, a_hi, b_tap + k * 2, b_hi, idesc, (c | tap | k) != 0 ? 1u : 0u);
            }
          }
          __syncwarp();
        } else {
#pragma unroll 1
          for (int tap = 0; tap < 9; ++tap) {
            mbar_wait(&b_full[sb], pb);
            tc_fence_after();
            const uint32_t b_tap = (smem_u32(b_smem + sb * Cfg::B_STAGE) >> 4) | (1u << 16);
            const uint32_t a_tap = a_lo0 + uint32_t(((tap / 3) * kHalo + (tap % 3)) * ROWB) / 16;
            if (elect_one()) {
#pragma unroll
              for (int k = 0; k < KC / 16; ++k)
                umma2_bf16_ss(d0, a_tap + k * 2, a_hi, b_tap + k * 2, b_hi, idesc, (c | tap | k) != 0 ? 1u : 0u);
              tc_commit2(&b_empty[sb]);
            }
            __syncwarp();
            if (++sb == SB) { sb = 0; pb ^= 1; }
          }
        }
        if (elect_one()) tc_commit2(&a_empty[sa]);
        __syncwarp();
        if (++sa == SA) { sa = 0; pa ^= 1; }
      }
      if (elect_one()) tc_commit2(&acc_full[as]);
      __syncwarp();
    }
  } else if (warp >= kEpiWarp0) {
    const int q = warp & 3;
    const int mb = (warp - kEpiWarp0) >> 2;
    const int m = q * 32 + lane;
    const int prow = m >> 3, pcol = (m & 7) + mb * 8;
    int it = 0;
    for (int u = pair_id; u < total_pairs; u += n_pairs, ++it) {
      int nt, tx, ty, img; bool dup;
      my_tile(u, nt, tx, ty, img, dup);
      const int as = it % NACC;
      const uint32_t aph = (it / NACC) & 1;
      const int y = ty * kTile + prow, x = tx * kTile + pcol;
      mbar_wait(&acc_full[as], aph);
      tc_fence_after();
      const uint32_t taddr = tmem_base + (uint32_t(q * 32) << 16) + as * (2 * BN) + mb * BN;
#pragma unroll 1
      for (int cc = 0; cc < BN / 32; ++cc) {
        uint32_t r[32];
        tmem_ld_32x32(taddr + cc * 32, r);
        tmem_ld_wait();
        if (cc == BN / 32 - 1) {
          tc_fence_before();
          __syncwarp();
          if (lane == 0) { if (leader) mbar_arrive(&acc_empty[as]); else mbar_arrive_remote(&acc_empty[as], 0); }
        }
        epilogue_bf16_chunk(p, r, epi_s + nt * BN + cc * 32, nt * BN + cc * 32, img, y, x, lane, !dup);
      }
    }
  }

  tc_fence_before();
  cluster.sync();
  if (warp == 2) {
    tc_fence_after();
    tmem_dealloc2(tmem_base, Cfg::TMEM_COLS);
  }
}

}
```

include/pnp_b200.h:

```cpp
#ifndef PNP_B200_H_
#define PNP_B200_H_

#include <stddef.h>
#include <stdint.h>

#ifdef __cplusplus
extern "C" {
#endif

typedef struct pnp_unet_plan pnp_unet_plan;

int pnp_init(void);
const char* pnp_last_error(void);
int pnp_num_sms(void);
int pnp_abi_version(void);

int pnp_psnr(const float* x, const float* gt, long long gt_batch_stride, float* out, int B, int HW, void* stream);

int pnp_psnr_allgather(const float* x, const float* gt, long long gt_batch_stride, float* out_local,
                       const unsigned long long* peer_base, int rank, int world, int slot_floats, int parity,
                       int flag_word, unsigned int* local_count, unsigned int count_target, unsigned int flag_target,
                       int* err_flag, int B, int HW, void* stream);

size_t pnp_ssim_workspace_bytes(int B, int H, int W);
int pnp_ssim(const float* x, const float* gt, long long gt_batch_stride, float* out, void* workspace, int B, int H, int W,
             void* stream);

int pnp_fft2c(const void* src_c64, void* dst_c64, int B, int H, int W, int inverse, void* stream);

int pnp_simulate_measurements(const float* gt, long long gt_batch_stride, const uint8_t* mask, long long mask_batch_stride,
                              const float* sigma_n, int sigma_stride, const unsigned long long* seeds,
                              void* y0_out_c64, void* x0_out_c64, void* aty0_out_c64, int B, int H, int W, void* stream);

int pnp_cartesian_masks(const int* accel, int accel_stride, const unsigned long long* seeds, int acs_cols, uint8_t* mask_out,
                        int B, int H, int W, void* stream);

int pnp_radial_masks(const double* frac, int frac_stride, const unsigned long long* seeds, uint8_t* mask_out,
                     int* lines_out, int B, int H, int W, void* stream);

int pnp_variable_density_masks(const int* accel, int accel_stride, const unsigned long long* seeds, int acs_h, int acs_w,
                               int power, uint8_t* mask_out, int B, int H, int W, void* stream);

int pnp_residual_real(const void* z_c64, const void* u_c64, float* v, long long n, void* stream);

size_t pnp_prox_workspace_bytes(int B, int H, int W);
int pnp_prox_dual(const float* x, const void* u_in_c64, const void* y0_c64, const uint8_t* mask,
                  long long mask_batch_stride, const float* mu, int mu_stride, void* z_out_c64, void* u_out_c64,
                  float* v_next, void* workspace, int B, int H, int W, void* stream);

int pnp_prox_prepared_supported(int H, int W);
int pnp_prox_prepared_bytes(int B, int H, int W, size_t* y0p_bytes, size_t* maskp_bytes);
int pnp_prox_prepare(const void* y0_c64, const uint8_t* mask, long long mask_batch_stride, void* y0T_c64, uint8_t* maskT,
                     int B, int H, int W, void* stream);
int pnp_prox_dual_prepared(const float* x, const void* u_in_c64, const void* y0T_c64, const uint8_t* maskT,
                           long long mask_batch_stride, const float* mu, int mu_stride, void* z_out_c64,
                           void* u_out_c64, float* v_next, int B, int H, int W, void* stream);

int pnp_prox_prepared_kind_async(const uint8_t* maskT, long long mask_batch_stride, int B, int H, int W, int* kind_host,
                                 void* stream);
int pnp_prox_dual_prepared_kind(const float* x, const void* u_in_c64, const void* y0T_c64, const uint8_t* maskT,
                                long long mask_batch_stride, const float* mu, int mu_stride, void* z_out_c64,
                                void* u_out_c64, float* v_next, int B, int H, int W, int kind, void* stream);

size_t pnp_unet_num_params(void);
size_t pnp_unet_packed_bytes(void);
int pnp_unet_pack_weights(const float* flat_params, void* packed, void* stream);
size_t pnp_unet_workspace_bytes(int B, int H, int W);
int pnp_unet_plan_create(pnp_unet_plan** plan, const void* packed, void* workspace, size_t workspace_bytes, int B,
                         int H, int W);
void pnp_unet_plan_destroy(pnp_unet_plan* plan);
int pnp_unet_forward(pnp_unet_plan* plan, const float* v, const float* sigma, float* x_out, float* preclamp,
                     void* stream);
int pnp_unet_profile(pnp_unet_plan* plan, const float* v, const float* sigma, float* x_out, void* stream, float* ms,
                     int* kinds, int* ids, int* n_inout);
int pnp_unet_num_launches(const pnp_unet_plan* plan);
int pnp_unet_micro_batch(const pnp_unet_plan* plan);
size_t pnp_unet_set_workspace_cap(size_t bytes);
int pnp_unet_set_splitk(int mode);
int pnp_unet_plan_tensor(const pnp_unet_plan* plan, const char* name, size_t* byte_offset, int* C, int* H, int* W);

size_t pnp_conv3x3_packed_bytes(int Cin, int Cout);
int pnp_conv3x3_bf16(const void* in0, int C0, const void* in1, int C1, const float* weights, const float* bias,
                     void* out, void* scratch, int B, int H, int W, int Cout, void* stream);

size_t pnp_policy_packed_floats(int n_time, int n_task);
int pnp_policy_step(const float* packed, const float* rtg, const float* emb, float* act, const long long* timesteps,
                    const long long* task, const long long* pos, float* act_out, float* rtg_out, float scale0, float scale1,
                    float scale2, int B, int K, int n_time, int n_task, void* stream);

size_t pnp_policy_encoder_packed_floats(void);
int pnp_policy_observe(const float* enc_packed, const float* x, int H, int W, const float* next_rtg, float* rtg, float* emb,
                       float* act, long long* timesteps, const long long* pos, const long long* t_dev, int B, int K,
                       int n_time, void* stream);

int pnp_step(pnp_unet_plan* plan, const float* v, const float* sigma, const void* u_in_c64, const void* y0_c64,
             const uint8_t* mask, long long mask_batch_stride, const float* mu, int mu_stride, float* x_out,
             void* z_out_c64, void* u_out_c64, float* v_next, void* prox_workspace, void* stream);

int pnp_step_prepared(pnp_unet_plan* plan, const float* v, const float* sigma, const void* u_in_c64,
                      const void* y0T_c64, const uint8_t* maskT, long long mask_batch_stride, const float* mu,
                      int mu_stride, float* x_out, void* z_out_c64, void* u_out_c64, float* v_next, void* stream);

int pnp_step_prepared_kind(pnp_unet_plan* plan, const float* v, const float* sigma, const void* u_in_c64,
                           const void* y0T_c64, const uint8_t* maskT, long long mask_batch_stride, const float* mu,
                           int mu_stride, float* x_out, void* z_out_c64, void* u_out_c64, float* v_next, int kind,
                           void* stream);

int pnp_step_prepared_active(pnp_unet_plan* plan, const float* v, const float* sigma, const void* u_in_c64,
                             const void* y0T_c64, const uint8_t* maskT, long long mask_batch_stride, const float* mu,
                             int mu_stride, float* x_out, void* z_out_c64, void* u_out_c64, float* v_next, int kind,
                             const uint8_t* active, void* stream);

#ifdef __cplusplus
}
#endif
#endif
```

Before: 25540.

## Chain consecutive pair-conv layers into one persistent launch with per-image readiness counters

Consecutive chainable UMMA pair convolutions (KC=64, BN=128, bf16 epilogue) are merged into a single persistent cluster kernel. The kernel walks a global item space spanning up to nine layers, and producers wait on per-image release/acquire counters set by the previous layer's epilogue warps. This targets launch gaps and tail-wave idle time between layers by letting later layers start on images whose inputs are complete. In exchange, chained layers stream their weights instead of keeping them resident in shared memory, and the scheme adds spin-waits with a timeout, a mapped host error word and a last-block counter reset. A grid-wide dependency like this could deadlock if not all clusters are co-resident.

```diff
diff --git a/dt4image_restoration_b200/_lib.py b/dt4image_restoration_b200/_lib.py
--- a/dt4image_restoration_b200/_lib.py
+++ b/dt4image_restoration_b200/_lib.py
@@ -62,6 +62,7 @@
     "pnp_unet_micro_batch": (c_int, [c_void_p]),
     "pnp_unet_set_workspace_cap": (c_size_t, [c_size_t]),
     "pnp_unet_set_splitk": (c_int, [c_int]),
+    "pnp_unet_set_chain": (c_int, [c_int]),
     "pnp_unet_plan_tensor": (c_int, [c_void_p, c_char_p, C.POINTER(c_size_t), C.POINTER(c_int), C.POINTER(c_int),
                                      C.POINTER(c_int)]),
     "pnp_conv3x3_packed_bytes": (c_size_t, [c_int, c_int]),
diff --git a/dt4image_restoration_b200/csrc/api.cu b/dt4image_restoration_b200/csrc/api.cu
--- a/dt4image_restoration_b200/csrc/api.cu
+++ b/dt4image_restoration_b200/csrc/api.cu
@@ -363,6 +363,7 @@
 }
 
 int pnp_unet_set_splitk(int mode) { return unet_set_splitk(mode); }
+int pnp_unet_set_chain(int mode) { return unet_set_chain(mode); }
 
 int pnp_unet_plan_tensor(const pnp_unet_plan* plan, const char* name, size_t* byte_offset, int* C, int* H, int* W) {
   if (!plan || !name) return -1;
diff --git a/dt4image_restoration_b200/csrc/pnp_internal.h b/dt4image_restoration_b200/csrc/pnp_internal.h
--- a/dt4image_restoration_b200/csrc/pnp_internal.h
+++ b/dt4image_restoration_b200/csrc/pnp_internal.h
@@ -69,6 +69,7 @@
                  int* ids, int* n_inout);
 int unet_num_launches(const UnetPlan* p);
 int unet_set_splitk(int mode);
+int unet_set_chain(int mode);
 size_t conv_packed_bytes(int Cin, int Cout);
 int conv3x3_single(const __nv_bfloat16* in0, int C0, const __nv_bfloat16* in1, int C1, const float* w_fp32,
                    const float* bias, __nv_bfloat16* out, uint8_t* wpk_scratch, int B, int H, int W, int Cout,
diff --git a/dt4image_restoration_b200/csrc/unet.cu b/dt4image_restoration_b200/csrc/unet.cu
--- a/dt4image_restoration_b200/csrc/unet.cu
+++ b/dt4image_restoration_b200/csrc/unet.cu
@@ -280,6 +280,12 @@
   if (mode >= -1 && mode <= 1) g_splitk_mode = mode;
   return old;
 }
+static int g_chain_mode = -1;
+int unet_set_chain(int mode) {
+  const int old = g_chain_mode;
+  if (mode >= -1 && mode <= 1) g_chain_mode = mode;
+  return old;
+}
 
 static const int kConvSmemMax = 227 * 1024;
 static const int kConvSmemBudget = 222 * 1024;
@@ -308,9 +314,11 @@
   rc |= set_conv_attr<32, 64, EPI_BF16>();
   rc |= set_conv_attr<64, 64, EPI_BF16>();
   rc |= set_conv_attr<64, 128, EPI_BF16>();
-  rc |= int(cudaFuncSetAttribute(conv3x3_pair_kernel<32, 64>, cudaFuncAttributeMaxDynamicSharedMemorySize, kConvSmemMax));
-  rc |= int(cudaFuncSetAttribute(conv3x3_pair_kernel<64, 64>, cudaFuncAttributeMaxDynamicSharedMemorySize, kConvSmemMax));
-  rc |= int(cudaFuncSetAttribute(conv3x3_pair_kernel<64, 128>, cudaFuncAttributeMaxDynamicSharedMemorySize, kConvSmemMax));
+  rc |= int(cudaFuncSetAttribute(conv3x3_pair_kernel<32, 64, 1>, cudaFuncAttributeMaxDynamicSharedMemorySize, kConvSmemMax));
+  rc |= int(cudaFuncSetAttribute(conv3x3_pair_kernel<64, 64, 1>, cudaFuncAttributeMaxDynamicSharedMemorySize, kConvSmemMax));
+  rc |= int(cudaFuncSetAttribute(conv3x3_pair_kernel<64, 128, 1>, cudaFuncAttributeMaxDynamicSharedMemorySize, kConvSmemMax));
+  rc |= int(cudaFuncSetAttribute(conv3x3_pair_kernel<64, 128, kMaxChain>, cudaFuncAttributeMaxDynamicSharedMemorySize,
+                                 kConvSmemMax));
   rc |= int(cudaFuncSetAttribute(conv3x3_kws_kernel, cudaFuncAttributeMaxDynamicSharedMemorySize, kConvSmemMax));
   rc |= int(cudaFuncSetAttribute(conv3x3_splitk_kernel, cudaFuncAttributeMaxDynamicSharedMemorySize, kSkSmem));
   if (rc) set_error("cudaFuncSetAttribute(MaxDynamicSharedMemorySize) failed");
@@ -356,7 +364,7 @@
   return n_tiles == 1 && wbytes + 3 * halo_stage_bytes(KC) <= kConvRingBytes;
 }
 
-static void size_rings(ConvLaunch& L) {
+static void size_rings(ConvLaunch& L, bool stream = false) {
   if (L.kws) {
     const int bar = KwsCfg::BAR_BYTES;
     const int avail = kConvSmemBudget - 1024 - bar - 1024;
@@ -376,7 +384,7 @@
   const int nchunks = L.p.nchunks0 + L.p.nchunks1;
   const int wtotal = nchunks * 9 * b_bytes;
   ConvParams& p = L.p;
-  if (weights_fit(L.KC, p.n_tiles, wtotal)) {
+  if (!stream && weights_fit(L.KC, p.n_tiles, wtotal)) {
     p.wres = 1;
     p.sb = 1;
     int sa = (avail - wtotal) / a_stage;
@@ -511,12 +519,15 @@
     return int(cudaLaunchKernelEx(&cfg, conv3x3_splitk_kernel, L.p, L.tm0, L.tm1));
   }
   if (L.pair) {
+    PairChain<1> ch{};
+    ch.L[0].tmA0 = L.tm0; ch.L[0].tmA1 = L.tm1; ch.L[0].tmW = L.tmw; ch.L[0].p = L.p;
+    ch.n_layers = 1; ch.total_items = L.p.total_tiles;
     if (L.KC == 32 && L.BN == 64)
-      launch_k(conv3x3_pair_kernel<32, 64>, dim3(L.grid), dim3(kConvThreads), size_t(L.smem), st, L.p, L.tm0, L.tm1, L.tmw);
+      launch_k(conv3x3_pair_kernel<32, 64, 1>, dim3(L.grid), dim3(kConvThreads), size_t(L.smem), st, ch);
     else if (L.KC == 64 && L.BN == 64)
-      launch_k(conv3x3_pair_kernel<64, 64>, dim3(L.grid), dim3(kConvThreads), size_t(L.smem), st, L.p, L.tm0, L.tm1, L.tmw);
+      launch_k(conv3x3_pair_kernel<64, 64, 1>, dim3(L.grid), dim3(kConvThreads), size_t(L.smem), st, ch);
     else if (L.KC == 64 && L.BN == 128)
-      launch_k(conv3x3_pair_kernel<64, 128>, dim3(L.grid), dim3(kConvThreads), size_t(L.smem), st, L.p, L.tm0, L.tm1, L.tmw);
+      launch_k(conv3x3_pair_kernel<64, 128, 1>, dim3(L.grid), dim3(kConvThreads), size_t(L.smem), st, ch);
     else { set_error("conv: unsupported (KC,BN) combination for the pair kernel"); return -4; }
     return int(cudaGetLastError());
   }
@@ -564,7 +575,7 @@
 
 struct TensorSlot { size_t off; int C, H, W; };
 
-enum { K_FIRST = 0, K_UMMA = 1, K_UPS = 3 };
+enum { K_FIRST = 0, K_UMMA = 1, K_UPS = 3, K_CHAIN = 4 };
 
 struct Op {
   int kind;
@@ -572,6 +583,12 @@
   int level;
   int conv;
   int rev;
+};
+
+struct ChainLaunch {
+  PairChain<kMaxChain> ch;
+  int count;
+  int grid, smem;
 };
 
 struct UnetPlan {
@@ -582,7 +599,10 @@
   const uint8_t* wts;
   TensorSlot tA[5], tB[5], skip[5], pooled[5], ups[4];
   std::vector<ConvLaunch> convs;
+  std::vector<ChainLaunch> chains;
   std::vector<Op> ops;
+  uint32_t* chain_sync;
+  int* chain_err;
   FirstConvW first;
 };
 
@@ -650,11 +670,76 @@
   return off;
 }
 
+static const int kChainDoneWords = 16;
+static size_t chain_sync_bytes(int B) { return (size_t(4) * (kChainDoneWords + 27 * size_t(B)) + 1023) / 1024 * 1024; }
+
 size_t unet_workspace_bytes(int B, int H, int W) {
   UnetPlan P{};
   P.B = B; P.H = H; P.W = W;
   for (int l = 0; l < 5; ++l) { P.Hl[l] = H >> l; P.Wl[l] = W >> l; }
-  return plan_layout(&P);
+  return plan_layout(&P) + chain_sync_bytes(B);
+}
+
+static bool chainable(const ConvLaunch& c, int clusters) {
+  return c.pair && !c.splitk && c.KC == 64 && c.BN == 128 && c.EPI == EPI_BF16 && c.p.total_tiles >= clusters;
+}
+
+static int form_chains(UnetPlan* P) {
+  int clusters = 0;
+  for (const ConvLaunch& c : P->convs) {
+    if (!(c.pair && !c.splitk && c.KC == 64 && c.BN == 128)) continue;
+    ConvLaunch streamed = c;
+    size_rings(streamed, true);
+    cudaLaunchConfig_t cfg{};
+    cfg.gridDim = dim3(g_num_sms); cfg.blockDim = dim3(kConvThreads); cfg.dynamicSmemBytes = size_t(streamed.smem);
+    cudaError_t err = cudaOccupancyMaxActiveClusters(&clusters, conv3x3_pair_kernel<64, 128, kMaxChain>, &cfg);
+    if (err != cudaSuccess || clusters < 1) { set_error("unet plan: cluster occupancy query failed"); return -4; }
+    clusters = std::min(clusters, g_num_sms / 2);
+    break;
+  }
+  if (!clusters) return 0;
+  std::vector<Op> ops;
+  for (size_t i = 0; i < P->ops.size();) {
+    size_t e = i;
+    auto conv_at = [&](size_t k) -> const ConvLaunch* {
+      return (k < P->ops.size() && P->ops[k].kind == K_UMMA) ? &P->convs[P->ops[k].conv] : nullptr;
+    };
+    const ConvLaunch* c0 = conv_at(i);
+    if (c0 && chainable(*c0, clusters))
+      while (e + 1 < P->ops.size() && int(e + 1 - i) < kMaxChain) {
+        const ConvLaunch* c = conv_at(e + 1);
+        if (!c || !chainable(*c, clusters)) break;
+        ++e;
+      }
+    if (e == i) { ops.push_back(P->ops[i++]); continue; }
+    if (P->chains.size() >= size_t(kChainDoneWords)) { set_error("unet plan: too many chains"); return -4; }
+    ChainLaunch cl{};
+    cl.count = int(e - i + 1);
+    PairChain<kMaxChain>& ch = cl.ch;
+    ch.n_layers = cl.count;
+    ch.done = P->chain_sync + P->chains.size();
+    ch.err = P->chain_err;
+    int items = 0;
+    for (int j = 0; j < cl.count; ++j) {
+      ConvLaunch& c = P->convs[P->ops[i + j].conv];
+      c.p.rev = 0;
+      size_rings(c, true);
+      cl.smem = c.smem;
+      PairLayer& L = ch.L[j];
+      L.tmA0 = c.tm0; L.tmA1 = c.tm1; L.tmW = c.tmw; L.p = c.p;
+      L.item0 = items;
+      L.ready = P->chain_sync + kChainDoneWords + size_t(P->ops[i + j].id) * P->B;
+      L.target = uint32_t(c.p.tiles_x * c.p.tiles_y * c.p.n_tiles * kNumEpiWarps);
+      items += c.p.total_tiles;
+    }
+    ch.total_items = items;
+    cl.grid = 2 * std::min(items, clusters);
+    ops.push_back(Op{K_CHAIN, 300 + P->ops[i].id, P->ops[e].level, int(P->chains.size())});
+    P->chains.push_back(cl);
+    i = e + 1;
+  }
+  P->ops.swap(ops);
+  return 0;
 }
 
 int unet_plan_create(UnetPlan** out, const uint8_t* packed, uint8_t* workspace, size_t workspace_bytes, int B, int H,
@@ -663,12 +748,14 @@
   UnetPlan* P = new UnetPlan();
   P->B = B; P->H = H; P->W = W;
   for (int l = 0; l < 5; ++l) { P->Hl[l] = H >> l; P->Wl[l] = W >> l; }
-  const size_t need = plan_layout(P);
+  const size_t need = plan_layout(P) + chain_sync_bytes(B);
   if (workspace_bytes < need) { delete P; set_error("unet plan: workspace too small"); return -5; }
   if ((reinterpret_cast<uintptr_t>(workspace) & 1023) || (reinterpret_cast<uintptr_t>(packed) & 1023)) {
     delete P; set_error("unet plan: workspace / packed weights must be 1024-byte aligned"); return -6;
   }
   P->ws = workspace; P->ws_bytes = workspace_bytes; P->wts = packed;
+  P->chain_sync = reinterpret_cast<uint32_t*>(
+      (reinterpret_cast<uintptr_t>(workspace) + workspace_bytes - chain_sync_bytes(B)) & ~uintptr_t(1023));
   LayerDesc L[27]; size_t ow, ob, n, pk;
   layer_table(L, ow, ob, n, pk);
   const float* flat = reinterpret_cast<const float*>(packed + pk);
@@ -723,19 +810,36 @@
     conv(blk * 3 + 2, P->tB[l], nullptr, P->tA[l], l);
   }
   if (rc) { delete P; return rc; }
+  if (g_chain_mode != 0) {
+    cudaError_t e = cudaHostAlloc(reinterpret_cast<void**>(&P->chain_err), sizeof(int), cudaHostAllocMapped);
+    if (e != cudaSuccess) { P->chain_err = nullptr; delete P; set_error("unet plan: cannot allocate the chain error word"); return int(e); }
+    *P->chain_err = 0;
+    rc = form_chains(P);
+    if (!rc && P->chains.empty()) { cudaFreeHost(P->chain_err); P->chain_err = nullptr; }
+    if (!rc && !P->chains.empty()) {
+      e = cudaMemset(P->chain_sync, 0, chain_sync_bytes(B));
+      if (e == cudaSuccess) e = cudaDeviceSynchronize();
+      if (e != cudaSuccess) { set_error("unet plan: cannot clear the chain counters"); rc = int(e); }
+    }
+    if (rc) { unet_plan_destroy(P); return rc; }
+  }
   {
-    int k = 0;
+    int r = 0;
     for (Op& op : P->ops) {
-      op.rev = k & 1;
+      if (op.kind == K_CHAIN) { op.rev = 0; r = 1; continue; }
+      op.rev = r;
+      r ^= 1;
       if (op.kind == K_UMMA) P->convs[op.conv].p.rev = op.rev;
-      ++k;
     }
   }
   *out = P;
   return 0;
 }
 
-void unet_plan_destroy(UnetPlan* P) { delete P; }
+void unet_plan_destroy(UnetPlan* P) {
+  if (P && P->chain_err) cudaFreeHost(P->chain_err);
+  delete P;
+}
 
 int unet_plan_tensor(const UnetPlan* P, const char* name, size_t* off, int* C, int* H, int* W) {
   const TensorSlot* s = nullptr;
@@ -780,6 +884,10 @@
   layer_table(L, ow, ob, n, pk);
   auto T = [&](const TensorSlot& s) { return reinterpret_cast<__nv_bfloat16*>(P->ws + s.off); };
   int rc = 0;
+  if (P->chain_err && *reinterpret_cast<volatile int*>(P->chain_err)) {
+    set_error("unet: a chained conv launch timed out waiting for its inputs (readiness protocol error)");
+    return -8;
+  }
   for (const Op& op : P->ops) {
     if (prof) prof->begin();
     switch (op.kind) {
@@ -796,6 +904,12 @@
         ConvLaunch& cl = P->convs[op.conv];
         if (cl.EPI == EPI_FINAL) { cl.p.noisy = v; cl.p.x_out = x_out; cl.p.preclamp = preclamp; cl.p.active = active; }
         rc = launch_conv(cl, st);
+        break;
+      }
+      case K_CHAIN: {
+        const ChainLaunch& cl = P->chains[op.conv];
+        launch_k(conv3x3_pair_kernel<64, 128, kMaxChain>, dim3(cl.grid), dim3(kConvThreads), size_t(cl.smem), st, cl.ch);
+        rc = int(cudaGetLastError());
         break;
       }
       case K_UPS: {
@@ -846,7 +960,7 @@
   for (int i = 0; i < n && i < cap; ++i) {
     float t = 0.f;
     cudaEventElapsedTime(&t, prof.ev[2 * i], prof.ev[2 * i + 1]);
-    ms[i] = t; kinds[i] = P->ops[i].kind; ids[i] = P->ops[i].id;
+    ms[i] = t; kinds[i] = P->ops[i].kind == K_CHAIN ? int(K_UMMA) : P->ops[i].kind; ids[i] = P->ops[i].id;
   }
   for (cudaEvent_t evt : prof.ev) cudaEventDestroy(evt);
   *n_inout = n < cap ? n : cap;
diff --git a/dt4image_restoration_b200/csrc/unet_conv_pair.cuh b/dt4image_restoration_b200/csrc/unet_conv_pair.cuh
--- a/dt4image_restoration_b200/csrc/unet_conv_pair.cuh
+++ b/dt4image_restoration_b200/csrc/unet_conv_pair.cuh
@@ -75,16 +75,54 @@
   static_assert((BN / 2) % 8 == 0, "half blobs must be whole 8-row groups");
 };
 
-template <int KC, int BN>
+__device__ __forceinline__ uint32_t ld_acquire_gpu(const uint32_t* p) {
+  uint32_t v;
+  asm volatile("ld.acquire.gpu.global.u32 %0, [%1];" : "=r"(v) : "l"(p) : "memory");
+  return v;
+}
+__device__ __forceinline__ void red_release_gpu_add(uint32_t* p, uint32_t v) {
+  asm volatile("red.release.gpu.global.add.u32 [%0], %1;" ::"l"(p), "r"(v) : "memory");
+}
+__device__ __forceinline__ uint64_t global_timer_ns() {
+  uint64_t t;
+  asm volatile("mov.u64 %0, %%globaltimer;" : "=l"(t));
+  return t;
+}
+__device__ __forceinline__ void fence_proxy_async_global() { asm volatile("fence.proxy.async.global;" ::: "memory"); }
+__device__ __forceinline__ void epi_bar_sync() { asm volatile("bar.sync 1, %0;" ::"r"(kNumEpiWarps * 32) : "memory"); }
+
+struct PairLayer {
+  CUtensorMap tmA0, tmA1;
+  CUtensorMap tmW;
+  ConvParams p;
+  int item0;
+  uint32_t* ready;
+  uint32_t target;
+};
+
+constexpr int kMaxChain = 9;
+
+template <int NL>
+struct PairChain {
+  PairLayer L[NL];
+  int n_layers;
+  int total_items;
+  uint32_t* done;
+  int* err;
+};
+
+constexpr uint64_t kReadyTimeoutNs = 4000000000ull;
+
+template <int KC, int BN, int NL>
 __global__ void __cluster_dims__(2, 1, 1) __launch_bounds__(kConvThreads, 1)
-conv3x3_pair_kernel(const ConvParams p, const __grid_constant__ CUtensorMap tmA0,
-                    const __grid_constant__ CUtensorMap tmA1, const __grid_constant__ CUtensorMap tmW) {
+conv3x3_pair_kernel(const __grid_constant__ PairChain<NL> ch) {
   using Cfg = PairCfg<KC, BN>;
   constexpr int ROWB = Cfg::ROWB;
   constexpr int NACC = Cfg::NACC;
-  const int SA = p.sa, SB = p.sb;
-  const int nchunks = p.nchunks0 + p.nchunks1;
-  const int b_region = p.wres ? nchunks * 9 * Cfg::B_BYTES : SB * Cfg::B_STAGE;
+  constexpr bool kChain = NL > 1;
+  const ConvParams& p0 = ch.L[0].p;
+  const int SA = p0.sa, SB = p0.sb;
+  const int b_region = p0.wres ? (p0.nchunks0 + p0.nchunks1) * 9 * Cfg::B_BYTES : SB * Cfg::B_STAGE;
 
   extern __shared__ uint8_t smem_raw[];
   uint8_t* smem = reinterpret_cast<uint8_t*>((reinterpret_cast<uintptr_t>(smem_raw) + 1023) & ~uintptr_t(1023));
@@ -106,15 +144,18 @@
   const bool leader = rank == 0;
   const int warp = threadIdx.x >> 5;
   const int lane = threadIdx.x & 31;
-  const int pixel_tiles = p.B * p.tiles_y * p.tiles_x;
-  const int total_pairs = p.total_tiles;
+  const int total_items = ch.total_items;
   const int pair_id = int(blockIdx.x) >> 1, n_pairs = int(gridDim.x) >> 1;
+  auto layer_of = [&](int g, int& j) {
+    if constexpr (kChain)
+      while (j + 1 < ch.n_layers && g >= ch.L[j + 1].item0) ++j;
+  };
 
   grid_dep_launch();
   if (warp == 0 && lane == 0) {
-    tma_prefetch_desc(&tmA0);
-    tma_prefetch_desc(&tmA1);
-    tma_prefetch_desc(&tmW);
+    tma_prefetch_desc(&ch.L[0].tmA0);
+    tma_prefetch_desc(&ch.L[0].tmA1);
+    tma_prefetch_desc(&ch.L[0].tmW);
   }
   if (warp == 1 && lane == 0) {
     for (int i = 0; i < SA; ++i) { mbar_init(&a_full[i], 1); mbar_init(&a_empty[i], kNumMmaWarps); }
@@ -127,7 +168,10 @@
     tmem_alloc2(tmem_slot, Cfg::TMEM_COLS);
     tmem_relinquish2();
   }
+  int epi_layer = 0;
   if (warp >= kEpiWarp0) {
+    layer_of(pair_id, epi_layer);
+    const ConvParams& p = ch.L[epi_layer].p;
     const int t = threadIdx.x - kEpiWarp0 * 32;
     for (int i = t; i < p.Cout; i += kNumEpiWarps * 32) epi_s[i] = __ldg(p.bias + i);
   }
@@ -136,8 +180,9 @@
   tc_fence_after();
   const uint32_t tmem_base = *tmem_slot;
 
-  auto my_tile = [&](int u, int& nt, int& tx, int& ty, int& img, bool& dup) {
-    const int uu = p.rev ? total_pairs - 1 - u : u;
+  auto my_tile = [&](const ConvParams& p, int u, int& nt, int& tx, int& ty, int& img, bool& dup) {
+    const int pixel_tiles = p.B * p.tiles_y * p.tiles_x;
+    const int uu = p.rev ? p.total_tiles - 1 - u : u;
     nt = uu % p.n_tiles;
     int pt = 2 * (uu / p.n_tiles) + int(rank);
     dup = pt >= pixel_tiles;
@@ -151,29 +196,48 @@
     if (lane == 0) {
       int sa = 0, pa = 0, sb = 0, pb = 0;
       const int row_half = int(rank) * (BN / 2);
-      if (p.wres && pair_id < total_pairs) {
+      if (p0.wres && pair_id < total_items) {
+        const int nchunks = p0.nchunks0 + p0.nchunks1;
         const uint32_t wbar = cluster_addr(w_full, 0);
         if (leader) mbar_arrive_expect_tx(w_full, 2u * uint32_t(nchunks) * 9 * Cfg::B_BYTES);
         for (int i = 0; i < nchunks * 9; ++i)
-          tma_load_2d_pair(b_smem + size_t(i) * Cfg::B_BYTES, &tmW, wbar, 0, i * BN + row_half);
+          tma_load_2d_pair(b_smem + size_t(i) * Cfg::B_BYTES, &ch.L[0].tmW, wbar, 0, i * BN + row_half);
       }
       grid_dep_wait();
-      for (int u = pair_id; u < total_pairs; u += n_pairs) {
+      bool timed_out = false;
+      int j = 0;
+      for (int g = pair_id; g < total_items; g += n_pairs) {
+        layer_of(g, j);
+        const PairLayer& Lj = ch.L[j];
+        const ConvParams& p = Lj.p;
         int nt, tx, ty, img; bool dup;
-        my_tile(u, nt, tx, ty, img, dup);
+        my_tile(p, g - Lj.item0, nt, tx, ty, img, dup);
+        if (kChain && j > 0) {
+          const uint32_t* ctr = ch.L[j - 1].ready + img;
+          const uint32_t need = ch.L[j - 1].target;
+          if (!timed_out && ld_acquire_gpu(ctr) < need) {
+            const uint64_t t0 = global_timer_ns();
+            while (ld_acquire_gpu(ctr) < need) {
+              if (global_timer_ns() - t0 > kReadyTimeoutNs) { timed_out = true; *reinterpret_cast<volatile int*>(ch.err) = 1; break; }
+              __nanosleep(64);
+            }
+          }
+          fence_proxy_async_global();
+        }
+        const int nchunks = p.nchunks0 + p.nchunks1;
         for (int c = 0; c < nchunks; ++c) {
           mbar_wait(&a_empty[sa], pa ^ 1);
           if (leader) mbar_arrive_expect_tx(&a_full[sa], 2u * Cfg::A_BYTES);
           const bool seg0 = c < p.nchunks0;
-          tma_load_4d_pair(a_smem + sa * Cfg::A_STAGE, seg0 ? &tmA0 : &tmA1, cluster_addr(&a_full[sa], 0),
+          tma_load_4d_pair(a_smem + sa * Cfg::A_STAGE, seg0 ? &Lj.tmA0 : &Lj.tmA1, cluster_addr(&a_full[sa], 0),
                            (seg0 ? c : c - p.nchunks0) * KC, tx * kTile - 1, ty * kTile - 1, img);
           if (++sa == SA) { sa = 0; pa ^= 1; }
-          if (p.wres) continue;
+          if (p0.wres) continue;
           const int row0 = (c * 9 * p.n_tiles + nt) * BN + row_half;
           for (int tap = 0; tap < 9; ++tap) {
             mbar_wait(&b_empty[sb], pb ^ 1);
             if (leader) mbar_arrive_expect_tx(&b_full[sb], 2u * Cfg::B_BYTES);
-            tma_load_2d_pair(b_smem + sb * Cfg::B_STAGE, &tmW, cluster_addr(&b_full[sb], 0), 0,
+            tma_load_2d_pair(b_smem + sb * Cfg::B_STAGE, &Lj.tmW, cluster_addr(&b_full[sb], 0), 0,
                              row0 + tap * p.n_tiles * BN);
             if (++sb == SB) { sb = 0; pb ^= 1; }
           }
@@ -187,9 +251,11 @@
     constexpr uint32_t a_hi = (uint32_t(kHalo * ROWB) >> 4) | (1u << 14) | (kLayout << 29);
     constexpr uint32_t b_hi = (uint32_t(8 * ROWB) >> 4) | (1u << 14) | (kLayout << 29);
     int sa = 0, pa = 0, sb = 0, pb = 0;
-    int it = 0;
-    if (p.wres && pair_id < total_pairs) mbar_wait(w_full, 0);
-    for (int u = pair_id; u < total_pairs; u += n_pairs, ++it) {
+    int it = 0, j = 0;
+    if (p0.wres && pair_id < total_items) mbar_wait(w_full, 0);
+    for (int g = pair_id; g < total_items; g += n_pairs, ++it) {
+      layer_of(g, j);
+      const int nchunks = ch.L[j].p.nchunks0 + ch.L[j].p.nchunks1;
       const int as = it % NACC;
       const uint32_t aph = (it / NACC) & 1;
       mbar_wait(&acc_empty[as], aph ^ 1);
@@ -198,7 +264,7 @@
         mbar_wait(&a_full[sa], pa);
         tc_fence_after();
         const uint32_t a_lo0 = ((smem_u32(a_smem + sa * Cfg::A_STAGE) + uint32_t(mb * 8 * ROWB)) >> 4) | (1u << 16);
-        if (p.wres) {
+        if (p0.wres) {
           const uint32_t b_lo0 = (smem_u32(b_smem + c * 9 * Cfg::B_BYTES) >> 4) | (1u << 16);
           if (elect_one()) {
 #pragma unroll
@@ -240,10 +306,20 @@
     const int mb = (warp - kEpiWarp0) >> 2;
     const int m = q * 32 + lane;
     const int prow = m >> 3, pcol = (m & 7) + mb * 8;
-    int it = 0;
-    for (int u = pair_id; u < total_pairs; u += n_pairs, ++it) {
+    int it = 0, j = 0;
+    for (int g = pair_id; g < total_items; g += n_pairs, ++it) {
+      layer_of(g, j);
+      const PairLayer& Lj = ch.L[j];
+      const ConvParams& p = Lj.p;
+      if (kChain && j != epi_layer) {
+        epi_bar_sync();
+        const int t = threadIdx.x - kEpiWarp0 * 32;
+        for (int i = t; i < p.Cout; i += kNumEpiWarps * 32) epi_s[i] = __ldg(p.bias + i);
+        epi_bar_sync();
+        epi_layer = j;
+      }
       int nt, tx, ty, img; bool dup;
-      my_tile(u, nt, tx, ty, img, dup);
+      my_tile(p, g - Lj.item0, nt, tx, ty, img, dup);
       const int as = it % NACC;
       const uint32_t aph = (it / NACC) & 1;
       const int y = ty * kTile + prow, x = tx * kTile + pcol;
@@ -262,6 +338,10 @@
         }
         epilogue_bf16_chunk(p, r, epi_s + nt * BN + cc * 32, nt * BN + cc * 32, img, y, x, lane, !dup);
       }
+      if (kChain && !dup && j + 1 < ch.n_layers) {
+        __syncwarp();
+        if (lane == 0) red_release_gpu_add(Lj.ready + img, 1u);
+      }
     }
   }
 
@@ -271,6 +351,20 @@
     tc_fence_after();
     tmem_dealloc2(tmem_base, Cfg::TMEM_COLS);
   }
-}
-
-}
+  if constexpr (kChain) {
+    uint32_t* last = tmem_slot + 1;
+    if (threadIdx.x == 0) {
+      __threadfence();
+      *last = atomicAdd(ch.done, 1u) == gridDim.x - 1 ? 1u : 0u;
+    }
+    __syncthreads();
+    if (*last) {
+      __threadfence();
+      for (int l = 0; l + 1 < ch.n_layers; ++l)
+        for (int i = threadIdx.x; i < ch.L[l].p.B; i += blockDim.x) ch.L[l].ready[i] = 0u;
+      if (threadIdx.x == 0) *ch.done = 0u;
+    }
+  }
+}
+
+}
diff --git a/include/pnp_b200.h b/include/pnp_b200.h
--- a/include/pnp_b200.h
+++ b/include/pnp_b200.h
@@ -77,6 +77,7 @@
 int pnp_unet_micro_batch(const pnp_unet_plan* plan);
 size_t pnp_unet_set_workspace_cap(size_t bytes);
 int pnp_unet_set_splitk(int mode);
+int pnp_unet_set_chain(int mode);
 int pnp_unet_plan_tensor(const pnp_unet_plan* plan, const char* name, size_t* byte_offset, int* C, int* H, int* W);
 
 size_t pnp_conv3x3_packed_bytes(int Cin, int Cout);
```

New measurement: 25860, median of 6. Within noise of the previous version (+1.2%).
